# jagannatharjun/AntiZ

Measured on AMD Instinct MI355X. Metric: input MB/s precompressed (1 GB synthetic, 100k streams) at 1/2/4/8 MI355X, higher is better.
Workload: dtype u8

## Files before the change

antiz_amd/__init__.py:

```python
import ctypes as C
import os

HERE = os.path.dirname(os.path.abspath(__file__))
LIB_PATH = os.environ.get("ATZ_LIB") or os.path.join(HERE, "_build", "libatz_accel.so")
CLI_PATH = os.path.join(HERE, "_build", "uncomp")

u64 = C.c_uint64
u8p = C.POINTER(C.c_uint8)


class Opts(C.Structure):
    _fields_ = [("recomp_tresh", u64), ("sizediff_tresh", u64), ("shortcut_len", u64), ("mismatch_tol", u64),
                ("chunksize", u64), ("brute_window", C.c_int32), ("device", C.c_int32)]


class Cand(C.Structure):
    _fields_ = [("offset", u64), ("comp_len", u64), ("infl_len", u64), ("type", C.c_int32), ("flags", C.c_uint32)]


class Result(C.Structure):
    _fields_ = [("clevel", C.c_uint8), ("window", C.c_uint8), ("memlevel", C.c_uint8), ("recomp", C.c_uint8),
                ("n_trials", C.c_uint32), ("ident", u64), ("first_diff", C.c_int64), ("n_diff", u64),
                ("diff_index", u64)]


class Stats(C.Structure):
    _fields_ = [(k, u64) for k in ("file_bytes", "n_streams", "n_recomp", "n_trials", "n_trials_shortcut",
                                   "n_rounds", "atz_bytes", "n_candidates", "n_continuations", "n_hazard")] + \
               [(k, C.c_double) for k in ("scan_ms", "sweep_ms", "write_ms", "total_ms", "k_trial_ms",
                                          "k_inflate_ms", "k_chains_ms", "k_other_ms")] + \
               [(k, u64) for k in ("k_trial_launches", "k_inflate_launches", "k_chains_launches",
                                   "k_trial_alg_bytes", "k_inflate_alg_bytes", "k_chains_alg_bytes",
                                   "trial_parsed_bytes")] + \
               [("k_match_ms", C.c_double)] + \
               [(k, u64) for k in ("k_match_launches", "k_match_positions", "n_trials_rerun", "n_fast_fallbacks",
                                   "trial_cyc_total", "trial_cyc_tree", "trial_cyc_emit", "trial_blocks",
                                   "trial_cyc_heap", "trial_cyc_fallback", "trial_symbols",
                                   "n_trials_speculative", "n_reinflated", "n_inflate_retries", "n_trials_replayed", "n_replay_checked",
                                   "n_trials_duplicate", "n_fast_restarts", "dev_bytes_peak", "dev_bytes_held",
                                   "n_trials_skipped")]

    def as_dict(self):
        return {k: getattr(self, k) for k, _ in self._fields_}


EXPORTS = ["atz_open", "atz_close", "atz_strerror", "atz_free", "atz_default_opts", "atz_scan", "atz_sweep",
           "atz_precompress", "atz_precompress_device", "atz_reconstruct", "atz_deflate", "atz_deflate_batch",
           "atz_inflate_batch", "atz_deflate_bound", "atz_shard_scan", "atz_shard_sweep", "atz_shard_piece",
           "atz_shard_assemble", "atz_reconstruct_device", "atz_deflate_batch_ex", "atz_set_strategies",
           "atz_set_containers", "atz_container_anchors"]

STRATEGIES = {"filtered": 1, "huffman": 2, "rle": 3}


def strategy_mask(names):
    if isinstance(names, str):
        names = [w for w in names.split(",") if w]
    mask = 0
    for w in names:
        if w not in STRATEGIES:
            raise ValueError("unknown strategy %r (known: %s)" % (w, ", ".join(sorted(STRATEGIES))))
        mask |= 1 << STRATEGIES[w]
    return mask


CONTAINERS = {"zip": 0, "gzip": 1}


def container_mask(names):
    if isinstance(names, str):
        names = [w for w in names.split(",") if w]
    mask = 0
    for w in names:
        if w not in CONTAINERS:
            raise ValueError("unknown container %r (known: %s)" % (w, ", ".join(sorted(CONTAINERS))))
        mask |= 1 << CONTAINERS[w]
    return mask


def pack_clevel(strategy, level, raw=False):
    if not (0 <= strategy <= 3 and 0 <= level <= 9) or (strategy >= 2 and level < 1):
        raise ValueError("strategy %d with level %d" % (strategy, level))
    return (int(bool(raw)) << 6) | (strategy << 4) | level


def unpack_clevel(b):
    return b >> 4, b & 15


def unpack_clevel3(b):
    return bool(b & 0x40), (b >> 4) & 3, b & 15

_lib = None


class AtzError(RuntimeError):

    def __init__(self, msg, code=0):
        super().__init__(msg)
        self.code = code


def lib():
    global _lib
    if _lib is None:
        if not os.path.exists(LIB_PATH):
            raise AtzError("libatz_accel.so not built: run `python -m antiz_amd.build` (no CPU fallback)")
        L = C.CDLL(LIB_PATH)
        L.atz_open.argtypes = [C.POINTER(C.c_void_p), C.POINTER(Opts)]
        L.atz_close.argtypes = [C.c_void_p]
        L.atz_strerror.restype = C.c_char_p
        L.atz_strerror.argtypes = [C.c_int]
        L.atz_free.argtypes = [C.c_void_p]
        L.atz_default_opts.argtypes = [C.POINTER(Opts)]
        L.atz_scan.argtypes = [C.c_void_p, C.c_char_p, u64, C.POINTER(C.POINTER(Cand)), C.POINTER(u64)]
        L.atz_sweep.argtypes = [C.c_void_p, C.POINTER(Cand), u64, C.POINTER(Result), C.POINTER(C.POINTER(u64)),
                                C.POINTER(u8p), C.POINTER(u64)]
        L.atz_precompress.argtypes = [C.c_void_p, C.c_char_p, u64, C.POINTER(u8p), C.POINTER(u64), C.POINTER(Stats)]
        L.atz_precompress_device.argtypes = [C.c_void_p, C.c_void_p, C.c_char_p, u64, C.POINTER(C.c_void_p),
                                             C.POINTER(u64), C.POINTER(Stats)]
        L.atz_reconstruct.argtypes = [C.c_void_p, C.c_char_p, u64, C.POINTER(u8p), C.POINTER(u64)]
        L.atz_deflate.argtypes = [C.c_void_p, C.c_char_p, u64, C.c_int, C.c_int, C.c_int, C.c_char_p, u64,
                                  C.POINTER(u64)]
        L.atz_inflate_batch.argtypes = [C.c_void_p, C.c_char_p, u64, C.POINTER(u64), C.POINTER(u64), u64,
                                        C.POINTER(C.c_uint32), C.POINTER(u64), C.POINTER(u64)]
        L.atz_deflate_batch.argtypes = [C.c_void_p, C.c_char_p, u64, C.POINTER(u64), C.POINTER(u64),
                                        C.POINTER(C.c_uint32), u64, C.c_char_p, C.POINTER(u64), C.POINTER(u64),
                                        C.POINTER(u64)]
        L.atz_deflate_batch_ex.argtypes = L.atz_deflate_batch.argtypes
        L.atz_set_strategies.argtypes = [C.c_void_p, C.c_uint32]
        L.atz_set_containers.argtypes = [C.c_void_p, C.c_uint32]
        L.atz_container_anchors.argtypes = [C.c_void_p, C.c_char_p, u64, C.c_uint32, C.POINTER(C.POINTER(u64)),
                                            C.POINTER(u64)]
        L.atz_deflate_bound.restype = u64
        L.atz_deflate_bound.argtypes = [u64, C.c_int, C.c_int]
        L.atz_shard_scan.argtypes = [C.c_void_p, C.c_void_p, C.c_char_p, u64, C.c_int, C.c_int, C.POINTER(u8p),
                                     C.POINTER(u64)]
        L.atz_shard_sweep.argtypes = [C.c_void_p, C.c_void_p, C.c_char_p, u64, C.POINTER(C.c_char_p),
                                      C.POINTER(u64), C.c_int, C.POINTER(u64), C.POINTER(u8p), C.POINTER(u64),
                                      C.POINTER(u64), C.POINTER(Stats)]
        L.atz_shard_piece.argtypes = [C.c_void_p, C.c_void_p]
        L.atz_reconstruct_device.argtypes = [C.c_void_p, C.c_void_p, C.c_char_p, u64, C.POINTER(C.c_void_p),
                                             C.POINTER(u64)]
        L.atz_shard_assemble.argtypes = [C.c_void_p, C.c_void_p, u64, C.c_char_p, u64, u64, u64, C.c_void_p, u64,
                                         C.POINTER(u64)]
        _lib = L
    return _lib


def _check(rc):
    if rc != 0:
        raise AtzError("atz error %d: %s" % (rc, lib().atz_strerror(rc).decode()), rc)


class Context:

    def __init__(self, recomp_tresh=128, sizediff_tresh=128, shortcut_len=512, mismatch_tol=2,
                 chunksize=524288, brute_window=False, device=-1, strategies=None, containers=None):
        L = lib()
        self.o = Opts(recomp_tresh, sizediff_tresh, shortcut_len, mismatch_tol, chunksize, int(brute_window), device)
        if strategies is None:
            strategies = os.environ.get("ATZ_STRATEGIES", "")
        mask = strategy_mask(strategies)
        if containers is None:
            containers = os.environ.get("ATZ_CONTAINERS", "")
        cmask = container_mask(containers)
        self.h = C.c_void_p()
        _check(L.atz_open(C.byref(self.h), C.byref(self.o)))
        if mask:
            _check(L.atz_set_strategies(self.h, mask))
        if cmask:
            _check(L.atz_set_containers(self.h, cmask))

    def close(self):
        if self.h:
            lib().atz_close(self.h)
            self.h = C.c_void_p()

    def __enter__(self):
        return self

    def __exit__(self, *a):
        self.close()

    def precompress(self, data):
        L = lib()
        p = u8p()
        n = u64(0)
        st = Stats()
        _check(L.atz_precompress(self.h, data, len(data), C.byref(p), C.byref(n), C.byref(st)))
        out = C.string_at(p, n.value)
        L.atz_free(p)
        return out, st.as_dict()
# ... 137 lines not shown
```

antiz_amd/csrc/atz_accel.cpp:

```cpp
#include "k_inflate.hip"
#include "k_deflate.hip"

#include <algorithm>
#include <array>
#include <chrono>
#include <cstdio>
#include <cstdlib>
#include <cstring>
#include <deque>
#include <string>
#include <memory>
#include <new>
#include <stdexcept>
#include <atomic>
#include <thread>
#include <condition_variable>
#include <mutex>
#include <functional>
#include <unordered_map>
#include <vector>
#include <dlfcn.h>
#include <signal.h>
#include <sys/time.h>
#include <ucontext.h>
// ... 164 lines not shown
    if (i < MAXS) pcs()[i] = (uint64_t)((ucontext_t*)uc)->uc_mcontext.gregs[REG_RIP] | ((uint64_t)slot << 56);
  }
  static void enroll() {
    if (!on().load() || my_slot() >= 0) return;
    std::lock_guard<std::mutex> lk(mu());
    const int k = nthr().load();
    if (k >= MAXT) return;
    thr()[k] = pthread_self();
    alive()[k] = true;
    my_slot() = k;
    nthr().store(k + 1);
  }
  static void leave() {
    if (my_slot() < 0) return;
    std::lock_guard<std::mutex> lk(mu());
    alive()[my_slot()] = false;
    my_slot() = -1;
  }
  struct Enroll { Enroll() { enroll(); } ~Enroll() { leave(); } };
  const char* path = nullptr;
  std::thread sampler;
  std::atomic<bool> stop{false};
  HostProf() {
    path = std::getenv("ATZ_HOSTPROF");
    if (!path || !*path) { path = nullptr; return; }
    pcs();
    n().store(0);
    struct sigaction sa{};
    sa.sa_sigaction = on_sig;
    sa.sa_flags = SA_SIGINFO | SA_RESTART;
    sigemptyset(&sa.sa_mask);
    sigaction(SIGPROF, &sa, nullptr);
    {
      std::lock_guard<std::mutex> lk(mu());
      nthr().store(0);
    }
    on().store(true);
    enroll();
    sampler = std::thread([this] {
      while (!stop.load()) {
        {
          std::lock_guard<std::mutex> lk(mu());
          const int k = std::min(nthr().load(), MAXT);
          for (int i = 0; i < k; i++)
            if (alive()[i]) pthread_kill(thr()[i], SIGPROF);
        }
        std::this_thread::sleep_for(std::chrono::microseconds(100));
      }
    });
  }
  ~HostProf() {
    if (!path) return;
    stop.store(true);
    sampler.join();
    on().store(false);
    const size_t cnt = std::min(n().load(), MAXS);
    std::unordered_map<uint64_t, uint64_t> hist;
    for (size_t i = 0; i < cnt; i++) hist[pcs()[i]]++;
    FILE* f = std::fopen(path, "a");
    if (f) {
      std::fprintf(f, "# call: %zu samples, %d threads\n", cnt, nthr().load());
      for (const auto& kv : hist) {
        const uint64_t pc = kv.first & ((1ull << 56) - 1);
        Dl_info di{};
        if (dladdr((void*)(uintptr_t)pc, &di) && di.dli_fname)
          std::fprintf(f, "%llu %d %s 0x%llx %s\n", (unsigned long long)kv.second, (int)(kv.first >> 56), di.dli_fname,
                       (unsigned long long)(pc - (uint64_t)(uintptr_t)di.dli_fbase), di.dli_sname ? di.dli_sname : "?");
        else
          std::fprintf(f, "%llu %d ? 0x%llx ?\n", (unsigned long long)kv.second, (int)(kv.first >> 56), (unsigned long long)pc);
      }
      std::fclose(f);
    }
    leave();
    std::lock_guard<std::mutex> lk(mu());
    nthr().store(0);
  }
};

struct DBuf {
  void* p = nullptr;
  size_t n = 0;
  DBuf() = default;
  DBuf(const DBuf&) = delete;
  DBuf& operator=(const DBuf&) = delete;
  ~DBuf() { release(); }
  int reserve(size_t need) {
    if (need <= n) return 0;
    const auto t0 = std::chrono::steady_clock::now();
    release();
    size_t cap = need + need / 4 + 65536;
    const hipError_t e = hipMalloc(&p, cap);
    g_dev.n_alloc++;
    g_dev.alloc_us += (uint64_t)std::chrono::duration_cast<std::chrono::microseconds>(std::chrono::steady_clock::now() - t0).count();
    if (e != hipSuccess) { p = nullptr; return ATZ_E_NOMEM; }
    n = cap;
    g_dev.add(n);
    return 0;
  }
  void release() {
    if (p) { hipFree(p); g_dev.sub(n); g_dev.n_free++; }
    p = nullptr;
    n = 0;
  }
  template <typename T> T* as() const { return reinterpret_cast<T*>(p); }
};

struct PinBuf {
  void* p = nullptr;
  size_t n = 0;
  PinBuf() = default;
  PinBuf(const PinBuf&) = delete;
  PinBuf& operator=(const PinBuf&) = delete;
  ~PinBuf() { if (p) (void)hipHostFree(p); }
  int reserve(size_t need) {
    if (need <= n) return 0;
    const auto t0 = std::chrono::steady_clock::now();
    if (p) { (void)hipHostFree(p); g_dev.n_free++; }
    p = nullptr;
    n = 0;
    const hipError_t e = hipHostMalloc(&p, need, hipHostMallocDefault);
    g_dev.n_alloc++;
    g_dev.alloc_us += (uint64_t)std::chrono::duration_cast<std::chrono::microseconds>(std::chrono::steady_clock::now() - t0).count();
    if (e != hipSuccess) return ATZ_E_NOMEM;
    n = need;
    return 0;
  }
  template <typename T> T* as() const { return reinterpret_cast<T*>(p); }
};

struct Rec {
  uint64_t offset, comp_len, infl_len;
  int type;
  uint32_t flags;
  uint64_t arena_off = ~0ull;
  bool noshort = false;
  uint8_t mhint = 0;
};

struct StreamState {
  const std::vector<uint32_t>* list = nullptr;
  uint32_t idx = 0;
  uint32_t phase = 0;
  uint8_t c = 9, w = 15, m = 9;
  uint64_t ident = 0;
  int64_t first_diff = -1;
  std::vector<uint32_t> rawdiff;
  std::vector<uint8_t> diffval;
  uint32_t trials = 0;
  int32_t rp = -1;
  uint16_t rp_saved = 0, rp_busy = 0;
  uint8_t rp_win[10] = {};
  bool recomp = false;
  std::vector<std::array<uint16_t, 5>> xl;
};


uint32_t pk(int c, int w, int m) { return ((uint32_t)c << 16) | ((uint32_t)w << 8) | (uint32_t)m; }

void prange(std::vector<uint32_t>& l, int cmin, int cmax, int wmin, int wmax, int mmin, int mmax) {
  for (int w = wmax; w >= wmin; w--)
    for (int m = mmax; m >= mmin; m--)
      for (int c = cmax; c >= cmin; c--) l.push_back(pk(c, w, m));
}
void list_a(std::vector<uint32_t>& l, int type) {
  if (type >= 24) return;
  int w = 10 + type / 4;
  switch (type % 4) {
    case 0: l.push_back(pk(0, w, 8)); l.push_back(pk(1, w, 8)); l.push_back(pk(1, w, 9));
            prange(l, 1, 1, w, w, 1, 7); prange(l, 2, 9, w, w, 1, 9); break;
    case 1: prange(l, 2, 5, w, w, 8, 8); prange(l, 2, 5, w, w, 1, 7); prange(l, 2, 5, w, w, 9, 9);
            prange(l, 1, 1, w, w, 1, 9); prange(l, 6, 9, w, w, 1, 9); break;
    case 2: l.push_back(pk(6, w, 8)); l.push_back(pk(6, w, 9)); prange(l, 6, 6, w, w, 1, 7);
            prange(l, 1, 5, w, w, 1, 9); prange(l, 7, 9, w, w, 1, 9); break;
    default: prange(l, 7, 9, w, w, 8, 8); prange(l, 7, 9, w, w, 1, 7); prange(l, 7, 9, w, w, 9, 9);
             prange(l, 1, 6, w, w, 1, 9); break;
  }
}
void list_b(std::vector<uint32_t>& l, int type) {
  if (type >= 24) return;
  int w = 10 + type / 4;
  if (w == 10) prange(l, 1, 9, 11, 15, 1, 9);
  else if (w == 15) prange(l, 1, 9, 10, 14, 1, 9);
  else { prange(l, 1, 9, 10, w - 1, 1, 9); prange(l, 1, 9, w + 1, 15, 1, 9); }
}

const std::vector<uint32_t>& trial_list(int type, bool brute) {
  static const std::array<std::array<std::vector<uint32_t>, 27>, 2> L = [] {
    std::array<std::array<std::vector<uint32_t>, 27>, 2> t;
    for (int ty = 0; ty < 27; ty++) { list_a(t[0][ty], ty); list_b(t[1][ty], ty); }
    return t;
  }();
  return L[brute ? 1 : 0][type];
}

uint64_t bound(uint64_t n, int w, int m) {
  uint64_t complen = n + ((n + 7) >> 3) + ((n + 63) >> 6) + 5;
  if (w != 15 || m + 7 != 15) return complen + 6;
  return n + (n >> 12) + (n >> 14) + (n >> 25) + 13 - 6 + 6;
}

double ms_since(std::chrono::steady_clock::time_point t) {
  return std::chrono::duration<double, std::milli>(std::chrono::steady_clock::now() - t).count();
}

void make_tables(DeflTables& T) {
  static const int xlb[29] = {0,0,0,0,0,0,0,0,1,1,1,1,2,2,2,2,3,3,3,3,4,4,4,4,5,5,5,5,0};
  static const int xdb[30] = {0,0,0,0,1,1,2,2,3,3,4,4,5,5,6,6,7,7,8,8,9,9,10,10,11,11,12,12,13,13};
  std::memset(&T, 0, sizeof(T));
  int len = 0, code;
  for (code = 0; code < 28; code++) {
    T.lbase[code] = (uint16_t)len;
    for (int k = 0; k < (1 << xlb[code]); k++) T.lcode[len++] = (uint8_t)code;
  }
  T.lbase[28] = 0;
  T.lcode[255] = 28;
  int dist = 0;
  for (code = 0; code < 16; code++) {
    T.dbase[code] = (uint16_t)dist;
    for (int k = 0; k < (1 << xdb[code]); k++) T.dcode[dist++] = (uint8_t)code;
  }
  dist >>= 7;
  for (; code < 30; code++) {
    T.dbase[code] = (uint16_t)(dist << 7);
    for (int k = 0; k < (1 << (xdb[code] - 7)); k++) T.dcode[256 + dist++] = (uint8_t)code;
  }
  uint16_t blc[16] = {0};
  for (int n = 0; n < 288; n++) {
    T.st_llen[n] = n < 144 ? 8 : n < 256 ? 9 : n < 280 ? 7 : 8;
    blc[T.st_llen[n]]++;
  }
  uint16_t next[16];
  uint32_t c = 0;
  for (int b = 1; b <= 15; b++) { c = (c + blc[b - 1]) << 1; next[b] = (uint16_t)c; }
  auto rev = [](uint32_t v, int l) { uint32_t r = 0; for (int i = 0; i < l; i++) { r = (r << 1) | (v & 1); v >>= 1; } return r; };
  for (int n = 0; n < 288; n++) T.st_lcode[n] = (uint16_t)rev(next[T.st_llen[n]]++, T.st_llen[n]);
  for (int n = 0; n < 30; n++) { T.st_dlen[n] = 5; T.st_dcode[n] = (uint16_t)rev((uint32_t)n, 5); }
}

int header_type_host(unsigned b0, unsigned b1) {
  static const uint16_t H[24] = {0x2815, 0x2853, 0x2891, 0x28cf, 0x3811, 0x384f, 0x388d, 0x38cb,
                                 0x480d, 0x484b, 0x4889, 0x48c7, 0x5809, 0x5847, 0x5885, 0x58c3,
                                 0x6805, 0x6843, 0x6881, 0x68de, 0x7801, 0x785e, 0x789c, 0x78da};
  unsigned h = (b0 << 8) | b1;
  for (int t = 0; t < 24; t++) if (H[t] == h) return t;
  return -1;
}

const uint8_t* const INFL_BASE = nullptr;
uint32_t* const CHAIN_BASE = nullptr;

}

struct KTimer {
  std::vector<std::pair<hipEvent_t, hipEvent_t>> pending;
  std::vector<int> kind;
  std::vector<hipEvent_t> pool;
  hipEvent_t get() {
    if (!pool.empty()) { hipEvent_t e = pool.back(); pool.pop_back(); return e; }
    hipEvent_t e; (void)hipEventCreate(&e); return e;
  }
};

struct RpEntry {
  uint32_t reads_max = 0;
  uint64_t addr = 0;
  uint64_t tab = 0;
  uint32_t nsym = 0, flags = 0;
  uint8_t state = 0;
  uint8_t window = 0;
  uint8_t memlevel = 0;
};
struct DevArena {
  static constexpr uint64_t CHUNK = 1ull << 30;
  std::mutex mu;
  std::vector<std::unique_ptr<DBuf>> chunks;
  std::vector<std::pair<uint64_t, uint64_t>> span;
  std::unordered_map<uint64_t, std::vector<uint64_t>> freel;
  size_t cur = 0;
  uint64_t used = 0, total = 0, cap = 0;
  uint64_t reused = 0;
  static uint64_t cls(uint64_t bytes) { return (bytes + 4095) & ~4095ull; }
  void reset(uint64_t cap_) {
    std::lock_guard<std::mutex> lk(mu);
    cur = 0; used = 0; total = 0; cap = cap_; reused = 0;
    freel.clear();
  }
  void release(uint64_t a, uint64_t bytes) {
    std::lock_guard<std::mutex> lk(mu);
    freel[cls(bytes)].push_back(a);
  }
  uint64_t alloc(uint64_t bytes) {
    bytes = cls(bytes);
    std::lock_guard<std::mutex> lk(mu);
    auto it = freel.find(bytes);
    if (it != freel.end() && !it->second.empty()) {
      const uint64_t a = it->second.back();
      it->second.pop_back();
      reused += bytes;
      return a;
    }
    if (total + bytes > cap) return 0;
    while (cur < chunks.size() && used + bytes > chunks[cur]->n) { cur++; used = 0; }
    if (cur == chunks.size()) {
      auto b = std::make_unique<DBuf>();
      if (b->reserve(std::max(CHUNK, bytes)) != 0) { (void)hipGetLastError(); return 0; }
      span.push_back({(uint64_t)(uintptr_t)b->p, (uint64_t)(uintptr_t)b->p + b->n});
      chunks.push_back(std::move(b));
      used = 0;
    }
    const uint64_t a = (uint64_t)(uintptr_t)chunks[cur]->p + used;
    used += bytes;
    total += bytes;
    return a;
  }
  bool holds(uint64_t a, uint64_t len) {
    std::lock_guard<std::mutex> lk(mu);
    for (const auto& s : span)
      if (a >= s.first && a + len <= s.second) return true;
    return false;
  }
};
struct ChainBufs {
  DBuf d_cjobs, d_cjobs2, d_cjobs3, d_heads, d_heads2;
};
struct Pipe {
  hipStream_t st = nullptr;
  KTimer kt;
  atz_stats_t stats{};
  DBuf d_trials, d_tres, d_out, d_syms, d_R, d_mjobs, d_diffjobs, d_diffpos, d_diffval, d_diffcnt, d_djobs;
  DBuf d_stopj;
  uint32_t* stopj_cur = nullptr;
  uint32_t mw_cap = 2;
  std::vector<std::unique_ptr<DBuf>> d_chains;
  size_t chains_next = 0;
  ChainBufs cb;
  PinBuf stage;
  size_t stage_used = 0;
  uint64_t r_next = 0;
  hipEvent_t ev_built = nullptr;

  hipStream_t pst = nullptr;
  std::vector<std::pair<uint32_t, int>> tmp_chains;
  uint64_t diag_builds = 0;
  std::vector<std::pair<uint32_t, uint32_t>> diag_rt;
  std::vector<uint64_t> diag_path;
  std::vector<uint32_t> diag_ntr;
  std::vector<uint16_t> diag_need;
  std::vector<uint32_t> slot;
  int id = 0;
  double t_list = 0, t_chains = 0, t_trials = 0, t_apply = 0, t_copy = 0, t_sync = 0;
  uint64_t n_copy = 0, n_sync = 0;
  static constexpr int NPH = 13;
  double ph[NPH] = {}, ph_wait[NPH] = {};
  std::chrono::steady_clock::time_point lap_t;
  double lap_w = 0;
  void lap_start() { lap_t = std::chrono::steady_clock::now(); lap_w = t_copy + t_sync; }
  void lap(int i) {
    const auto n = std::chrono::steady_clock::now();
    ph[i] += std::chrono::duration<double, std::milli>(n - lap_t).count();
    ph_wait[i] += t_copy + t_sync - lap_w;
    lap_t = n;
    lap_w = t_copy + t_sync;
  }
  uint64_t kind[3][10][14] = {};
  ~Pipe() {
    if (ev_built) hipEventDestroy(ev_built);
    if (pst) { hipStreamSynchronize(pst); hipStreamDestroy(pst); }
    if (st) { hipStreamSynchronize(st); hipStreamDestroy(st); }
    for (hipEvent_t e : kt.pool) hipEventDestroy(e);
  }
};

struct TrialSet {
  std::vector<Trial> tr[3];
  std::vector<uint32_t> perm[3];
  std::vector<TrialRes> res[3];
  size_t base = 0;
};

struct atz_ctx {
  KTimer kt;
  atz_opts_t o{};
  int dev = 0;
  hipStream_t st = nullptr;
  DBuf d_rec, d_atzin;
  DBuf d_file, d_pos, d_cnt, d_hbase, d_jobs, d_res, d_virt, d_infl, d_chains, d_heads, d_streams, d_trials,
      d_tres, d_out, d_syms, d_adler, d_meta, d_segs, d_atz, d_diffjobs, d_diffpos, d_diffval, d_diffcnt,
      d_cjobs, d_cjobs2, d_cjobs3, d_heads2, d_tmp, d_R, d_mjobs, d_ins, d_arena, d_arena_used;
  std::vector<Rec> recs;
  std::vector<uint64_t> infl_off;
  std::vector<uint32_t> adler;
  const uint8_t* hfile = nullptr;
  uint64_t flen = 0;
  bool scan_valid = false;
  uint32_t strat_mask = 0;
  uint32_t cont_mask = 0;
  bool exact_idents = false;
  std::vector<uint32_t> scan_trailer;
  bool file_on_device = false;
  const uint8_t* dev_file = nullptr;
  atz_stats_t stats{};
  std::vector<std::array<uint64_t, 10>> chain_off;
  DevArena chain_arena;
  DevArena rp_arena;
  std::vector<std::array<RpEntry, 9>> rp_pool;
  std::mutex rp_mu;
  PinBuf depth_pin;
  struct Sched {
    std::mutex mu;
    std::condition_variable cv;
    std::vector<std::deque<uint32_t>> q;
    std::vector<size_t> unfinished;
    bool closed = false;
    bool abort = false;
    std::atomic<size_t> published{0};
  } sched;
  std::vector<std::unique_ptr<Pipe>> pipes;
  std::vector<std::unique_ptr<DBuf>> slabs;
  size_t pipes_running = 1;
  size_t sweep_nmax = 0;
  std::atomic<bool> sweep_abort{false};
  std::shared_ptr<struct ScanState> scan_keep;
  std::function<void(uint64_t)> on_records;
  std::vector<StreamState> ss_keep;
  std::vector<StreamDev> sd_keep;
  struct Shard {
    std::shared_ptr<struct ScanState> S;
    int rank = -1, world = 0;
    uint32_t ja = 0, jb = 0;
    uint64_t F = 0;
    std::vector<std::pair<uint64_t, uint64_t>> all;
    uint64_t piece_len = 0;
    int stage = 0;
    std::chrono::steady_clock::time_point t0;
  } shard;
};

template <class C>
static void kbeg(C* c, int kind, hipStream_t st = nullptr) {
  hipEvent_t a = c->kt.get(), b = c->kt.get();
  (void)hipEventRecord(a, st ? st : c->st);
  c->kt.pending.push_back({a, b});
  c->kt.kind.push_back(kind);
}
template <class C>
static void kend(C* c, hipStream_t st = nullptr) { (void)hipEventRecord(c->kt.pending.back().second, st ? st : c->st); }
template <class C>
static void kcollect(C* c) {
  for (size_t i = 0; i < c->kt.pending.size(); i++) {
    float ms = 0;
    (void)hipEventElapsedTime(&ms, c->kt.pending[i].first, c->kt.pending[i].second);
    switch (c->kt.kind[i]) {
      case 0: c->stats.k_trial_ms += ms; c->stats.k_trial_launches++; break;
      case 1: c->stats.k_inflate_ms += ms; c->stats.k_inflate_launches++; break;
      case 2: c->stats.k_chains_ms += ms; c->stats.k_chains_launches++; break;
      case 4: c->stats.k_match_ms += ms; c->stats.k_match_launches++; break;
      default: c->stats.k_other_ms += ms; break;
    }
    c->kt.pool.push_back(c->kt.pending[i].first);
    c->kt.pool.push_back(c->kt.pending[i].second);
  }
  c->kt.pending.clear();
  c->kt.kind.clear();
}

template <class C> static void copy_timed(C*, double) {}
template <> void copy_timed<Pipe>(Pipe* p, double ms) { p->t_copy += ms; p->n_copy++; }
static bool stage_on() {
  static const bool v = [] { const char* e = std::getenv("ATZ_STAGE"); return !e || std::atoi(e) != 0; }();
  return v;
}
static constexpr size_t STAGE_BYTES = 32u << 20;
template <class C> static const void* staged(C*, const void* h, size_t) { return h; }
template <> const void* staged<Pipe>(Pipe* p, const void* h, size_t n) {
  if (!stage_on() || !n) return h;
  if (!p->stage.p && p->stage.reserve(STAGE_BYTES)) return h;
  const size_t a = (p->stage_used + 255) & ~(size_t)255;
  if (a + n > p->stage.n) return h;
  std::memcpy(static_cast<uint8_t*>(p->stage.p) + a, h, n);
  p->stage_used = a + n;
  return static_cast<uint8_t*>(p->stage.p) + a;
}
static hipError_t pipe_sync(Pipe* p) {
  const auto t = std::chrono::steady_clock::now();
  const hipError_t e = hipStreamSynchronize(p->st);
  if (e == hipSuccess) p->stage_used = 0;
  p->t_sync += std::chrono::duration<double, std::milli>(std::chrono::steady_clock::now() - t).count();
  p->n_sync++;
  return e;
}
static hipError_t pipe_copy(Pipe* p, void* dst, const void* src, size_t n, hipMemcpyKind k) {
  const auto t = std::chrono::steady_clock::now();
  if (k == hipMemcpyHostToDevice) src = staged(p, src, n);
  const hipError_t e = hipMemcpyAsync(dst, src, n, k, p->st);
  copy_timed(p, std::chrono::duration<double, std::milli>(std::chrono::steady_clock::now() - t).count());
  return e;
}
template <class C>
static int upload(C* c, DBuf& b, const void* h, size_t n, size_t slack = 4096) {
  if (int r = b.reserve(n + slack)) return r;
  const auto t = std::chrono::steady_clock::now();
  if (n) HIPCHK(hipMemcpyAsync(b.p, staged(c, h, n), n, hipMemcpyHostToDevice, c->st));
  copy_timed(c, std::chrono::duration<double, std::milli>(std::chrono::steady_clock::now() - t).count());
  return 0;
}

static bool sync_debug() {
  static const int v = [] { const char* e = std::getenv("ATZ_SYNC_DEBUG"); return (int)(e && *e == '1'); }();
  return v == 1;
}
#define KCHECK(name)                                                                            \
  do {                                                                                          \
    hipError_t e_ = hipGetLastError();                                                          \
    if (e_ == hipSuccess && sync_debug()) e_ = hipStreamSynchronize(c->st);                     \
    if (e_ != hipSuccess) {                                                                     \
      std::fprintf(stderr, "atz: kernel %s failed: %s (%s:%d)\n", name, hipGetErrorString(e_), \
                   __FILE__, __LINE__);                                                         \
      return ATZ_E_HIP;                                                                         \
    }                                                                                           \
  } while (0)

struct Chunk {
  uint64_t co;
  uint64_t len;
  uint8_t b0;
  bool b0_file;
};

static constexpr uint64_t ARENA_SLOT = 65536;

static int timing_level() {
  static const int v = [] { const char* e = std::getenv("ATZ_TIMING"); return (int)(e ? std::atoi(e) : 0); }();
  return v;
}
static bool timing_on() { return timing_level() >= 1; }

static int run_inflate_jobs(atz_ctx* c, const uint8_t* d_in, uint8_t* d_out, const std::vector<InfJob>& jobs,
                            std::vector<InfRes>& res, uint64_t arena_cap = 0, bool full_ring = false,
                            bool arena_reset = true, bool raw = false) {
  res.resize(jobs.size());
  if (jobs.empty()) return 0;
  auto ti0 = std::chrono::steady_clock::now();
  if (int r = upload(c, c->d_jobs, jobs.data(), jobs.size() * sizeof(InfJob))) return r;
  if (int r = c->d_res.reserve(jobs.size() * sizeof(InfRes))) return r;
  if (int r = c->d_arena_used.reserve(64)) return r;
  if (arena_cap && arena_reset) {
    if (int r = c->d_arena.reserve(arena_cap)) return r;
    HIPCHK(hipMemsetAsync(c->d_arena_used.p, 0, 8, c->st));
  }
  uint32_t n = (uint32_t)jobs.size();
  bool small = !full_ring;
  for (const InfJob& jb : jobs) small = small && jb.out_off != NO_OUT;
  kbeg(c, 1);
  auto kern = small ? (raw ? k_inflate<INF_RING_SMALL, true> : k_inflate<INF_RING_SMALL>)
                    : (raw ? k_inflate<INF_RING_FULL, true> : k_inflate<INF_RING_FULL>);
  hipLaunchKernelGGL(kern, dim3(n), dim3(64), 0, c->st, d_in, d_out, c->d_jobs.as<InfJob>(), c->d_res.as<InfRes>(), n,
                     c->d_arena.as<uint8_t>(), c->d_arena_used.as<unsigned long long>(), arena_cap);
// ... 782 lines not shown
  }
  std::vector<ChainJob> nine, rest;
  for (const ChainJob& jb : big) ((jb.memlevel == 9 && jb.n < 65536) ? nine : rest).push_back(jb);
  big.swap(rest);
  if (!nine.empty()) {
    const size_t nbs = 4096;
    if (int r = B.d_heads2.reserve(nbs * 65536 * 4)) return r;
    std::vector<ChainJob>& pk = nine;
    for (size_t k = 0; k < pk.size(); k++) pk[k].slot = (uint32_t)(k % nbs);
    if (int r = upload(c, B.d_cjobs3, pk.data(), pk.size() * sizeof(ChainJob))) return r;
    for (size_t b0 = 0; b0 < pk.size();) {
      const size_t nb = std::min(nbs - b0 % nbs, pk.size() - b0);
      kbeg(c, 2);
      hipLaunchKernelGGL(k_buckets_pk<16>, dim3((uint32_t)nb), dim3(256), 0, c->st, INFL_BASE,
                         B.d_cjobs3.as<ChainJob>() + b0, chains, B.d_heads2.as<uint32_t>(),
                         (uint32_t)nb);
      kend(c);
      KCHECK("k_buckets_pk");
      b0 += nb;
    }
  }
  const size_t batch = 4096;
  if (!big.empty() && (int)B.d_heads.reserve(batch * 65536 * 8)) return ATZ_E_NOMEM;
  for (size_t k = 0; k < big.size(); k++) big[k].slot = (uint32_t)(k % batch);
  if (int r = upload(c, B.d_cjobs, big.data(), big.size() * sizeof(ChainJob))) return r;
  for (size_t b0 = 0; b0 < big.size(); b0 += batch) {
    size_t nb = std::min(batch, big.size() - b0);
    kbeg(c, 2);
    hipLaunchKernelGGL(k_buckets, dim3((uint32_t)nb), dim3(64), 0, c->st, INFL_BASE,
                       B.d_cjobs.as<ChainJob>() + b0, chains, B.d_heads.as<uint64_t>(),
                       (uint32_t)nb);
    kend(c);
    KCHECK("k_buckets");
  }
  for (const ChainJob& jb : jobs) c->stats.k_chains_alg_bytes += 9 * jb.n;
  return 0;
}

static void forget_tmp_chains(atz_ctx* x, Pipe* c) {
  for (auto& q : c->tmp_chains) x->chain_off[q.first][q.second] = ~0ull;
  c->tmp_chains.clear();
  c->chains_next = 0;
}
static int ensure_chains_on(atz_ctx* x, Pipe* c, const std::vector<std::pair<uint32_t, int>>& need, ChainBufs& B) {
  auto bytes = [&](uint32_t s) { return 8 * ((x->recs[s].infl_len + 63) & ~63ull); };
  std::vector<ChainJob> jobs;
  std::vector<size_t> tmp;
  uint64_t tmp_bytes = 0;
  for (auto& q : need) {
    uint32_t s = q.first;
    int m = q.second;
    if (x->chain_off[s][m] != ~0ull) continue;
    ChainJob jb;
    jb.infl_off = x->infl_off[s];
    jb.n = x->recs[s].infl_len;
    jb.memlevel = (uint32_t)m;
    jb.slot = 0;
    jb.dslot = 10 * s + (uint32_t)m;
    jb.pad_ = 0;
    const uint64_t a = x->chain_arena.alloc(bytes(s));
    if (a) {
      jb.chain_off = a >> 2;
    } else {
      jb.chain_off = tmp_bytes >> 2;
      tmp_bytes += (bytes(s) + 255) & ~255ull;
      tmp.push_back(jobs.size());
      c->tmp_chains.push_back({s, m});
    }
    x->chain_off[s][m] = jb.chain_off;
    jobs.push_back(jb);
    c->diag_builds++;
  }
  if (jobs.empty()) return 0;
  if (!tmp.empty()) {
    if (c->chains_next == c->d_chains.size()) c->d_chains.emplace_back(new DBuf());
    DBuf& tb = *c->d_chains[c->chains_next++];
    if (int r = tb.reserve(tmp_bytes + 4096)) return r;
    const uint64_t base = (uint64_t)(uintptr_t)tb.p >> 2;
    for (size_t k : tmp) {
      jobs[k].chain_off += base;
      x->chain_off[(uint32_t)(jobs[k].dslot / 10)][jobs[k].memlevel] = jobs[k].chain_off;
    }
  }
  if (int r = build_bucket_jobs(x, c, B, jobs, CHAIN_BASE, true, x->depth_pin.as<uint32_t>())) return r;
  if (bucket_verify()) {
    uint64_t tot = 0;
    std::vector<ChainJob> alt(jobs);
    for (ChainJob& jb : alt) { jb.chain_off = tot; tot += 2 * ((jb.n + 63) & ~63ull); }
    DBuf tmp;
    if (int r = tmp.reserve(tot * 4 + 4096)) return r;
    if (int r = build_bucket_jobs(x, c, B, alt, tmp.as<uint32_t>(), false, nullptr)) return r;
    std::vector<uint32_t> h1(tot), h2(tot);
    for (size_t k = 0; k < jobs.size(); k++)
      HIPCHK(hipMemcpyAsync(h1.data() + alt[k].chain_off, (const void*)(uintptr_t)(jobs[k].chain_off << 2),
                            8 * ((jobs[k].n + 63) & ~63ull), hipMemcpyDeviceToHost, c->st));
    HIPCHK(hipMemcpyAsync(h2.data(), tmp.p, tot * 4, hipMemcpyDeviceToHost, c->st));
    HIPCHK(hipStreamSynchronize(c->st));
    for (size_t k = 0; k < jobs.size(); k++) {
      const uint64_t npad = (alt[k].n + 63) & ~63ull, nh = alt[k].n >= 3 ? alt[k].n - 2 : 0;
      const uint32_t* a = h1.data() + alt[k].chain_off;
      const uint32_t* b2 = h2.data() + alt[k].chain_off;
      uint64_t start = 0, deepest = 0;
      for (uint64_t i = 0; i < nh; i++) {
        if (a[i] != b2[i] || a[npad + i] != b2[npad + i]) {
          std::fprintf(stderr, "atz: bucket mismatch: job %zu n %llu m %u at %llu\n", k, (unsigned long long)alt[k].n,
                       alt[k].memlevel, (unsigned long long)i);
          return ATZ_E_INTERNAL;
        }
        if (b2[npad + i] & BUCKET_FIRST) start = i;
        deepest = std::max(deepest, i - start);
      }
      const uint32_t dsort = x->depth_pin.p ? x->depth_pin.as<uint32_t>()[jobs[k].dslot] : 0u;
      if (x->depth_pin.p && nh && dsort != ~0u && dsort != deepest) {
        std::fprintf(stderr, "atz: deepest bucket mismatch: job %zu n %llu m %u: %u vs %llu\n", k,
                     (unsigned long long)alt[k].n, alt[k].memlevel, dsort, (unsigned long long)deepest);
        return ATZ_E_INTERNAL;
      }
    }
  }
  return 0;
}

static bool big_sweep(const atz_ctx* x) { return x->recs.size() > 16000 || x->pipes_running >= 6; }
static bool mhint_on(const atz_ctx* x) {
  static const int v = [] { const char* e = std::getenv("ATZ_MHINT"); return e ? std::atoi(e) : -1; }();
  return v < 0 ? big_sweep(x) : v != 0;
}
static uint64_t match_prefix(uint64_t n, int memlevel, bool big) {
  static const uint64_t mul = [] { const char* e = std::getenv("ATZ_PREFIX_MUL"); return e ? (uint64_t)std::max(1, std::atoi(e)) : 2ull; }();
  static const uint64_t lo = [] { const char* e = std::getenv("ATZ_PREFIX_MIN"); return e ? (uint64_t)std::max(64, std::atoi(e)) : 0ull; }();
  const uint64_t floor = lo ? lo : big ? 3072 : 1024;
  return std::min(n, std::max<uint64_t>(floor, mul << (memlevel + 6)));
}

static uint32_t lazy_host(uint32_t level) {
  return level == 7 ? 32u : level == 8 ? 128u : 258u;
}
static uint32_t nice_host(uint32_t level) {
  return level == 7 ? 128u : 258u;
}
static uint64_t c_cfg_host(uint32_t level) {
  static const uint16_t chain[10] = {0, 4, 8, 32, 16, 32, 128, 256, 1024, 4096};
  return chain[level < 10 ? level : 9];
}
static uint64_t match_win() {
  static const uint64_t v = [] { const char* e = std::getenv("ATZ_MATCH_WIN"); return e ? (uint64_t)std::atoll(e) : 16320ull; }();
  return v;
}
static uint64_t match_span(const MatchJob& m) {
  const uint64_t md = (1ull << m.window) - 262;
  const uint64_t lo = m.p0 > md ? (m.p0 - md) & ~3ull : 0ull;
  return std::min<uint64_t>(m.p1 + 258 + 24, m.n) - lo;
}
static int launch_match(atz_ctx* x, Pipe* c, const std::vector<MatchJob>& mj_in) {
  if (mj_in.empty()) return 0;
  static const uint64_t cls[] = {4096, 8192, 12288, 16384, 24576, 32768, 40960, 49152};
  constexpr int NC = 8;
  std::vector<MatchJob> cut;
  const bool win = match_win() > 0;
  if (win)
    for (const MatchJob& m : mj_in) {
      if (match_span(m) <= cls[NC - 1]) { cut.push_back(m); continue; }
      for (uint64_t a = m.p0; a < m.p1; a += std::min<uint64_t>(match_win(), 16320)) {
        MatchJob h = m;
        h.p0 = a;
        h.p1 = std::min<uint64_t>(m.p1, a + std::min<uint64_t>(match_win(), 16320));
        cut.push_back(h);
      }
    }
  const std::vector<MatchJob>& mj0 = win ? cut : mj_in;
  auto class_of = [&](const MatchJob& m) -> int {
    const uint64_t b = match_span(m);
    for (int k = 0; k < NC; k++) if (b <= cls[k] && (win || k < 6)) return k;
    return NC;
  };
  auto group_of = [](int k) -> int { return k; };
  std::vector<MatchJob> mj;
  mj.reserve(mj0.size());
  size_t cnt[NC + 1] = {};
  int gmax[NC + 1];
  for (int k = 0; k <= NC; k++) gmax[k] = -1;
  for (const MatchJob& m : mj0) {
    const int k = class_of(m), g = group_of(k);
    cnt[g]++;
    gmax[g] = std::max(gmax[g], k);
  }
  size_t beg[NC + 2] = {};
  for (int k = 0; k <= NC; k++) beg[k + 1] = beg[k] + cnt[k];
  mj.resize(mj0.size());
  {
    size_t at[NC + 1];
    for (int k = 0; k <= NC; k++) at[k] = beg[k];
    for (const MatchJob& m : mj0) mj[at[group_of(class_of(m))]++] = m;
    auto work = [](const MatchJob& m) -> uint64_t {
      const uint64_t chain = std::min<uint64_t>(c_cfg_host(m.level), (m.p1 >> (m.memlevel + 7)) + 1);
      return (m.p1 - m.p0) * chain;
    };
    for (int k = 0; k <= NC; k++)
      std::stable_sort(mj.begin() + beg[k], mj.begin() + beg[k + 1],
                       [&](const MatchJob& a, const MatchJob& b) { return work(a) > work(b); });
  }
  if (int r = upload(c, c->d_mjobs, mj.data(), mj.size() * sizeof(MatchJob))) return r;
  for (int k = 0; k <= NC; k++) {
    if (!cnt[k]) continue;
    kbeg(c, 4);
    if (k < NC)
      hipLaunchKernelGGL(k_match_lds, dim3((uint32_t)cnt[k]), dim3(MATCH_THREADS), (uint32_t)(3 * cls[gmax[k]] + 64), c->st,
                         INFL_BASE, CHAIN_BASE, c->d_R.as<uint2>(),
                         c->d_mjobs.as<MatchJob>() + beg[k]);
    else
      hipLaunchKernelGGL(k_match, dim3((uint32_t)cnt[k]), dim3(256), 0, c->st, INFL_BASE,
                         CHAIN_BASE, c->d_R.as<uint2>(), c->d_mjobs.as<MatchJob>() + beg[k]);
    kend(c);
    KCHECK("k_match");
  }
  for (const MatchJob& m : mj) c->stats.k_match_positions += m.p1 - m.p0;
  return 0;
}

static uint32_t mw_cap_for(size_t n_streams) {
  static const int v = [] { const char* e = std::getenv("ATZ_MW"); return (int)(e ? std::max(0, std::min(9, std::atoi(e))) : -1); }();
  return v >= 0 ? (uint32_t)v : n_streams <= 16000 ? 4u : 2u;
}
static bool mw_trial(const Pipe* c, int kind, uint32_t memlevel) { return kind != 0 && memlevel <= c->mw_cap; }
static uint32_t trial_variant(const Pipe* c, int k, const Trial& t) {
  return (mw_trial(c, k, t.memlevel) ? 1u : 0u) | ((t.host & TH_STRAT) << 1);
}
static uint64_t sym_words(const Pipe* c, int kind, uint32_t memlevel, uint64_t n) {
  return (mw_trial(c, kind, memlevel) ? n + 64 : 0) + (1ull << (memlevel + 6)) + 64;
}
struct TrialBatch {
  std::vector<Trial> tr[3];
  uint64_t out_tot = 0, sym_tot = 0;
  std::pair<int, uint32_t> add(const Pipe* c, uint32_t s, uint64_t len, int cl, int w, int m, uint32_t strat,
                               uint8_t mode, uint64_t best_ident) {
    if (strat == 1 && cl < 4) strat = 0;
    const int kind = cl == 0 || strat >= 2 ? 0 : cl <= 3 ? 1 : 2;
    Trial t{};
    t.stream = s; t.clevel = (uint8_t)cl; t.window = (uint8_t)w; t.memlevel = (uint8_t)m;
    t.mode = mode; t.host = strat;
    t.best_ident = best_ident;
    t.out_off = out_tot; t.out_cap = bound(len, w, m) + 64;
    out_tot += (t.out_cap + 255) & ~255ull;
    t.sym_off = sym_tot; sym_tot += sym_words(c, kind, (uint32_t)m, len);
    tr[kind].push_back(t);
    return {kind, (uint32_t)tr[kind].size() - 1};
  }
  int reserve(Pipe* c) const {
    if (int r = c->d_out.reserve(out_tot + 4096)) return r;
    return c->d_syms.reserve(sym_tot * 4 + 4096);
  }
};

static bool stopflag_on() {
  static const bool v = [] { const char* e = std::getenv("ATZ_STOPFLAG"); return !e || std::atoi(e) != 0; }();
  return v;
}
static void trials_order(atz_ctx* x, const Pipe* c, std::vector<Trial>* in, TrialSet& S) {
  for (int k = 0; k < 3; k++) {
    const size_t n = in[k].size();
    S.perm[k].resize(n);
    std::vector<uint64_t> key(n);
    const uint32_t mwm = c->mw_cap;
    const bool packed = n < (1u << 20);
    bool strat = false;
    for (size_t q = 0; q < n; q++) {
      const Trial& t = in[k][q];
      strat |= (t.host & TH_STRAT) != 0;
      const uint64_t w = x->recs[t.stream].infl_len * (uint64_t)(k == 1 ? 3 : 1) * (uint64_t)(10 - t.memlevel) *
                         (uint64_t)((t.mode & TM_REPLAY) ? 1 : 4);
      const uint64_t mw = k != 0 && t.memlevel <= mwm;
      const uint64_t jr = stopflag_on() ? 15 - std::min<uint32_t>(t.spec_j, 15) : 0;
      key[q] = packed ? (mw << 63) | (jr << 59) | (std::min<uint64_t>(w, (1ull << 39) - 1) << 20) | ((1u << 20) - 1 - q) : w;
      S.perm[k][q] = (uint32_t)q;
    }
    if (packed) {
      std::sort(key.begin(), key.end(), std::greater<uint64_t>());
      for (size_t q = 0; q < n; q++) S.perm[k][q] = (uint32_t)((1u << 20) - 1 - (key[q] & ((1u << 20) - 1)));
    } else {
      std::stable_sort(S.perm[k].begin(), S.perm[k].end(), [&](uint32_t a, uint32_t b) {
        const bool ma = mw_trial(c, k, in[k][a].memlevel), mb = mw_trial(c, k, in[k][b].memlevel);
        return ma != mb ? ma : key[a] > key[b];
      });
    }
    if (strat)
      std::stable_sort(S.perm[k].begin(), S.perm[k].end(), [&](uint32_t a, uint32_t b) {
        return trial_variant(c, k, in[k][a]) < trial_variant(c, k, in[k][b]);
      });
    S.tr[k].resize(n);
    for (size_t q = 0; q < n; q++) S.tr[k][q] = in[k][S.perm[k][q]];
    S.res[k].clear();
  }
  S.base = 0;
}
static int trials_launch(atz_ctx* x, Pipe* c, const uint8_t* d_cmp, const SweepOpts& so, int k, const Trial* h,
                         size_t cnt, size_t base) {
  struct Kern { int kind; uint32_t strat; bool mw; void (*fn)(SweepArgs); const char* name; };
  static const Kern kerns[] = {
      {0, 0, false, k_trial_stored, "k_trial_stored"},
      {0, 2, false, k_trial_huff, "k_trial_huff"},
      {0, 3, false, k_trial_rle, "k_trial_rle"},
      {1, 0, true, k_trial_fast_mw<BITMAP_BITS>, "k_trial_fast"},
      {1, 0, false, k_trial_fast<BITMAP_BITS>, "k_trial_fast"},
      {2, 0, true, k_trial_slow_mw, "k_trial_slow"},
      {2, 0, false, k_trial_slow, "k_trial_slow"},
      {2, 1, true, k_trial_slow_filt_mw, "k_trial_slow_filt"},
      {2, 1, false, k_trial_slow_filt, "k_trial_slow_filt"},
  };
  for (size_t i = 0; i < cnt; i++)
    if (h[i].host & (TH_WAITS | TH_DUP)) return ATZ_E_INTERNAL;
  for (size_t i = 0; i < cnt;) {
    const bool mw = mw_trial(c, k, h[i].memlevel);
    size_t j = i + 1;
    while (j < cnt && mw_trial(c, k, h[j].memlevel) == mw) j++;
    HIPCHK(pipe_copy(c, c->d_trials.as<Trial>() + base + i, h + i, (j - i) * sizeof(Trial), hipMemcpyHostToDevice));
    i = j;
  }
  auto launch1 = [&](const Trial* hh, size_t n1, size_t b1, uint32_t variant) -> int {
    (void)hh;
    const bool mw = variant & 1u;
    const Kern* kn = nullptr;
    for (const Kern& e : kerns)
      if (e.kind == k && e.strat == variant >> 1 && e.mw == mw) kn = &e;
    if (!kn) return ATZ_E_INTERNAL;
    SweepArgs A;
    A.file = d_cmp; A.infl = INFL_BASE; A.chains = CHAIN_BASE;
    A.R = c->d_R.as<uint2>();
    A.streams = x->d_streams.as<StreamDev>(); A.trials = c->d_trials.as<Trial>() + b1;
    A.res = c->d_tres.as<TrialRes>() + b1; A.out = c->d_out.as<uint8_t>(); A.syms = c->d_syms.as<uint32_t>();
    A.adler = x->d_adler.as<uint32_t>(); A.o = so; A.ntrials = (uint32_t)n1;
    A.stopj = c->stopj_cur;
    dim3 g((uint32_t)n1), b(mw ? MW_THREADS : 64);
    kbeg(c, 0);
    hipLaunchKernelGGL(kn->fn, g, b, 0, c->st, A);
    kend(c);
    KCHECK(kn->name);
    return 0;
  };
  size_t i = 0;
  while (i < cnt) {
    const uint32_t v = trial_variant(c, k, h[i]);
    size_t j = i + 1;
    while (j < cnt && trial_variant(c, k, h[j]) == v) j++;
    if (int r = launch1(h + i, j - i, base + i, v)) return r;
    i = j;
  }
  return 0;
}
static bool early_match_on() {
  static const bool v = [] { const char* e = std::getenv("ATZ_EARLY"); return !e || std::atoi(e) != 0; }();
  return v;
}
static MatchJob first_match_job(atz_ctx* x, Pipe* c, int k, Trial& t) {
  const uint64_t n = x->recs[t.stream].infl_len;
  t.r_off = c->r_next;
  c->r_next += ((n + 63) & ~63ull) + 256;
  t.x_lim = (t.mode & TM_FULL) || (mhint_on(x) && t.memlevel == x->recs[t.stream].mhint) ? n : match_prefix(n, t.memlevel, big_sweep(x));
  MatchJob m{};
  m.infl_off = x->infl_off[t.stream]; m.n = n; m.chain_off = t.chain_off; m.r_off = t.r_off;
  m.p0 = 0; m.p1 = t.x_lim; m.level = t.clevel; m.window = t.window; m.fast = k == 1; m.memlevel = t.memlevel;
  return m;
}
static int trials_first_launch(atz_ctx* x, Pipe* c, const uint8_t* d_cmp, TrialSet& S, const SweepOpts& so,
                               size_t bases[3]) {
  std::vector<Trial>* tr = S.tr;
  std::vector<TrialRes>* res = S.res;
  std::vector<MatchJob> mj;
  for (int k = 0; k < 3; k++)
    for (const Trial& t : tr[k])
      if (x->recs[t.stream].infl_len >= (1ull << 31)) {
        std::fprintf(stderr, "atz: stream of %llu inflated bytes exceeds the 2 GiB trial limit\n",
                     (unsigned long long)x->recs[t.stream].infl_len);
        return ATZ_E_ARG;
      }
  for (int k = 1; k < 3; k++)
    for (Trial& t : tr[k]) {
      const uint64_t n = x->recs[t.stream].infl_len;
      if (tm_unchecked_replay(t.mode)) { t.r_off = 0; t.x_lim = n; continue; }
      if (t.x_lim) continue;
      if (MatchJob m = first_match_job(x, c, k, t); m.p1 > m.p0) mj.push_back(m);
    }
  if (int r = c->d_R.reserve(c->r_next * sizeof(uint2) + 4096)) return r;
  c->lap(6);
  if (int r = launch_match(x, c, mj)) return r;
  c->lap(7);
  const size_t tot_trials = tr[0].size() + tr[1].size() + tr[2].size();
  if (int r = c->d_trials.reserve(2 * tot_trials * sizeof(Trial) + 64)) return r;
  if (int r = c->d_tres.reserve(2 * tot_trials * sizeof(TrialRes) + 64)) return r;
  size_t base = 0;
  for (int k = 0; k < 3; k++) {
    bases[k] = base;
    res[k].resize(tr[k].size());
    if (tr[k].empty()) continue;
    if (int r = trials_launch(x, c, d_cmp, so, k, tr[k].data(), tr[k].size(), base)) return r;
    base += tr[k].size();
  }
  S.base = base;
  c->lap(8);
  return 0;
}
static int trials_first_finish(Pipe* c, TrialSet& S, const size_t bases[3]);
static int trials_first(atz_ctx* x, Pipe* c, const uint8_t* d_cmp, TrialSet& S, const SweepOpts& so) {
  size_t bases[3];
  if (int r = trials_first_launch(x, c, d_cmp, S, so, bases)) return r;
  return trials_first_finish(c, S, bases);
}
static int trials_first_finish(Pipe* c, TrialSet& S, const size_t bases[3]) {
  std::vector<Trial>* tr = S.tr;
  std::vector<TrialRes>* res = S.res;
  for (int k = 0; k < 3; k++)
    if (!tr[k].empty())
      HIPCHK(pipe_copy(c, res[k].data(), c->d_tres.as<TrialRes>() + bases[k], tr[k].size() * sizeof(TrialRes), hipMemcpyDeviceToHost));
  HIPCHK(pipe_sync(c));
  kcollect(c);
  c->lap(9);
  return 0;
}
static int trials_rerun(atz_ctx* x, Pipe* c, const uint8_t* d_cmp, TrialSet& S, const SweepOpts& so,
                        const std::function<bool(const Trial&)>& want) {
  std::vector<Trial>* tr = S.tr;
  std::vector<TrialRes>* res = S.res;
  std::vector<Trial> again[3];
  std::vector<size_t> where[3];
  std::vector<MatchJob> mj;
  for (int k = 1; k < 3; k++)
    for (size_t q = 0; q < tr[k].size(); q++) {
      if (res[k][q].state != TR_NEED_R || (want && !want(tr[k][q]))) continue;
      Trial t = tr[k][q];
      const uint64_t n = x->recs[t.stream].infl_len;
      MatchJob m{};
      m.infl_off = x->infl_off[t.stream]; m.n = n; m.chain_off = t.chain_off; m.r_off = t.r_off;
      m.p0 = t.x_lim; m.p1 = n; m.level = t.clevel; m.window = t.window; m.fast = k == 1; m.memlevel = t.memlevel;
      if (m.p1 > m.p0) mj.push_back(m);
      t.x_lim = n;
      again[k].push_back(t);
      where[k].push_back(q);
      c->stats.n_trials_rerun++;
    }
  if (again[1].empty() && again[2].empty()) return 0;
  if (int r = launch_match(x, c, mj)) return r;
  std::vector<TrialRes> rr[3];
  size_t base = S.base, bases[3] = {0, 0, 0};
  if (base + again[1].size() + again[2].size() > 2 * (tr[0].size() + tr[1].size() + tr[2].size())) return ATZ_E_INTERNAL;
  for (int k = 1; k < 3; k++) {
    bases[k] = base;
    if (again[k].empty()) continue;
    if (int r = trials_launch(x, c, d_cmp, so, k, again[k].data(), again[k].size(), base)) return r;
    rr[k].resize(again[k].size());
    base += again[k].size();
  }
  for (int k = 1; k < 3; k++)
    if (!again[k].empty())
      HIPCHK(pipe_copy(c, rr[k].data(), c->d_tres.as<TrialRes>() + bases[k], again[k].size() * sizeof(TrialRes), hipMemcpyDeviceToHost));
  HIPCHK(pipe_sync(c));
  kcollect(c);
  for (int k = 1; k < 3; k++)
    for (size_t q = 0; q < again[k].size(); q++) {
      if (rr[k][q].state == TR_NEED_R) return ATZ_E_INTERNAL;
      res[k][where[k][q]] = rr[k][q];
      tr[k][where[k][q]].x_lim = again[k][q].x_lim;
    }
  S.base = base;
  return 0;
}
static void trials_results(const TrialSet& S, std::vector<TrialRes>* res) {
  for (int k = 0; k < 3; k++) {
    res[k].resize(S.tr[k].size());
    for (size_t q = 0; q < S.tr[k].size(); q++) res[k][S.perm[k][q]] = S.res[k][q];
  }
}
static int run_trials(atz_ctx* x, Pipe* c, const uint8_t* d_cmp, std::vector<Trial>* tr, const SweepOpts& so,
                      std::vector<TrialRes>* res) {
  TrialSet S;
  trials_order(x, c, tr, S);
  c->r_next = 0;
  if (int r = trials_first(x, c, d_cmp, S, so)) return r;
  if (int r = trials_rerun(x, c, d_cmp, S, so, nullptr)) return r;
  trials_results(S, res);
  return 0;
}

static int replay_mode() {
  static const int v = [] { const char* e = std::getenv("ATZ_REPLAY"); return (int)(e ? std::atoi(e) : 1); }();
  return v;
}
static bool replay_on() { return replay_mode() != 0; }
static constexpr uint64_t RP_ARENA_CAP = 24ull << 30;

static bool dedup_on() {
  static const int v = [] { const char* e = std::getenv("ATZ_DEDUP"); return (int)(e ? std::atoi(e) : 1); }();
  return v != 0;
}
static void replay_from(Trial& t, const RpEntry& e, bool bf) {
  if (bf) {
    t.mode |= TM_REPLAY;
    const uint32_t lm = std::min<uint32_t>(e.memlevel, t.memlevel);
    if (dedup_on() && (uint64_t)e.nsym + 2 <= (1ull << (lm + 6))) t.host |= TH_DUP;
  } else if (e.tab) {
    t.mode |= TM_REPLAY | TM_CHECKED;
    t.rp_tab = e.tab;
  } else {
    return;
  }
  t.rp_syms = e.addr; t.rp_nsym = e.nsym; t.rp_flags = e.flags;
}
static bool budget_free(atz_ctx* x, int kind, const Trial& t) {
  const uint32_t Bq = (uint32_t)(c_cfg_host(t.clevel) >> (kind == 1 ? 0 : 2));
  return x->depth_pin.as<uint32_t>()[10 * (size_t)t.stream + t.memlevel] <= Bq;
}
static bool replay_free(atz_ctx* x, int kind, const Trial& t) {
  return x->recs[t.stream].infl_len <= (1ull << t.window) - 262 && budget_free(x, kind, t);
}

static bool budget_free(atz_ctx* x, int kind, const Trial& t);
static void level_dups(atz_ctx* x, std::vector<StreamState>& ss, std::vector<Trial>& slow) {
  for (Trial& t : slow) {
    if (t.clevel < 7 || t.clevel > 9 || (t.mode & TM_FULL)) continue;
    const StreamState& st = ss[t.stream];
    for (const auto& r : st.xl) {
      if (r[0] != t.window || r[1] != t.memlevel || r[2] <= t.clevel) continue;
      if (r[3] < lazy_host(t.clevel) && r[4] < nice_host(t.clevel) && budget_free(x, 2, t)) t.host |= TH_DUP;
      break;
    }
  }
}
template <class Mine>
static void level_record(atz_ctx* x, std::vector<StreamState>& ss, const std::vector<Trial>& slow,
                         const std::vector<TrialRes>& res, const Mine& mine) {
  for (size_t q = 0; q < slow.size(); q++) {
    const Trial& t = slow[q];
    const TrialRes& r = res[q];
    if (!mine(t.stream)) continue;
    if (t.clevel < 7 || t.clevel > 9 || (t.host & TH_DUP) || r.state == TR_NEED_R || r.state == TR_OVERFLOW ||
        r.state == TR_SKIPPED)
      continue;
    if (!budget_free(x, 2, t)) continue;
    StreamState& st = ss[t.stream];
    bool have = false;
    for (const auto& e : st.xl) have |= e[0] == t.window && e[1] == t.memlevel;
    if (have) continue;
    uint32_t rm = r.reads_max;
    if (r.saved_flags & 4) {
      if (st.rp < 0) continue;
      rm = x->rp_pool[st.rp][t.clevel - 1].reads_max;
    }
    st.xl.push_back({(uint16_t)t.window, (uint16_t)t.memlevel, (uint16_t)t.clevel, (uint16_t)(rm >> 16),
                     (uint16_t)(rm & 0xffffu)});
  }
}

static void plan_replay(atz_ctx* x, Pipe* c, std::vector<StreamState>& ss, int kind, std::vector<Trial>& trs,
                        std::vector<std::array<uint32_t, 4>>& savers) {
  const bool checked = replay_mode() != 3 && kind == 2;
  for (size_t q = 0; q < trs.size(); q++) {
    Trial& t = trs[q];
    if (t.clevel < 1 || t.clevel > 9 || (t.mode & TM_FULL) || (t.host & TH_DUP)) continue;
    const uint64_t n = x->recs[t.stream].infl_len;
    const uint64_t wsz = 1ull << t.window;
    if (n > wsz + (wsz - 262)) continue;
    const bool bf = replay_free(x, kind, t);
    if (!bf && !checked) continue;
    StreamState& st = ss[t.stream];
    const uint32_t L = t.clevel;
    const bool saved = (st.rp_saved >> L) & 1u, busy = (st.rp_busy >> L) & 1u;
    const bool same_w = st.rp_win[L] == t.window;
    if (saved && same_w) {
      if (replay_mode() == 2) continue;
      replay_from(t, x->rp_pool[st.rp][L - 1], bf);
    } else if (busy && same_w && replay_mode() != 2 && (bf || x->rp_pool[st.rp][L - 1].tab)) {
      t.host |= TH_WAITS;
    } else if (!saved && !busy && bf) {
      if (st.rp < 0) {
        std::lock_guard<std::mutex> lk(x->rp_mu);
        if (x->rp_pool.size() == x->rp_pool.capacity()) continue;
        st.rp = (int32_t)x->rp_pool.size();
        x->rp_pool.emplace_back();
      }
      RpEntry& e = x->rp_pool[st.rp][L - 1];
      const uint64_t sb = (4 * (n + 64) + 255) & ~255ull, tb = kind == 2 ? ((8 * n + 255) & ~255ull) : 0;
      if (!e.addr) {
        e.addr = x->rp_arena.alloc(sb + tb);
        if (!e.addr) continue;
        e.tab = tb ? e.addr + sb : 0;
      }
      e.state = 1;
// ... 13 lines not shown
  static const bool on = [] { const char* e = std::getenv("ATZ_ELIG"); return !e || std::atoi(e) != 0; }();
  if (!on || x->exact_idents || x->o.mismatch_tol > x->o.recomp_tresh || C <= x->o.recomp_tresh) return 0;
  return C - x->o.recomp_tresh - 1;
}

static constexpr uint64_t ROUND_BUDGET_BYTES = 24ull << 30;

static bool sched_take(atz_ctx* x, int g, std::vector<uint32_t>& batch) {
  auto& Q = x->sched;
  std::unique_lock<std::mutex> lk(Q.mu);
  batch.clear();
  auto stop = [&] { return Q.abort || x->sweep_abort.load(std::memory_order_relaxed); };
  std::deque<uint32_t>& q = Q.q[g];
  Q.cv.wait(lk, [&] { return stop() || !q.empty() || (Q.closed && Q.unfinished[g] == 0); });
  if (stop() || q.empty()) return false;
  batch.assign(q.begin(), q.end());
  q.clear();
  return true;
}
static void sched_give(atz_ctx* x, int g, const std::vector<StreamState>& ss, const std::vector<uint32_t>& active,
                       const std::vector<uint32_t>& waiting) {
  auto& Q = x->sched;
  std::lock_guard<std::mutex> lk(Q.mu);
  std::vector<uint32_t> front(waiting);
  size_t done = 0;
  for (uint32_t s : active) { if (ss[s].phase == 2) done++; else front.push_back(s); }
  Q.unfinished[g] -= done;
  Q.q[g].insert(Q.q[g].begin(), front.begin(), front.end());
  Q.cv.notify_all();
}
static void sched_abort(atz_ctx* x) {
  std::lock_guard<std::mutex> lk(x->sched.mu);
  x->sched.abort = true;
  x->sched.cv.notify_all();
}

static size_t round_target(const atz_ctx* x);
static void account_trial(atz_ctx* x, Pipe* c, int k, const Trial& t, const TrialRes& r) {
  const uint64_t C = x->recs[t.stream].comp_len;
  c->stats.trial_parsed_bytes += r.parsed;
  c->stats.n_fast_fallbacks += r.fallbacks & 0xffffffffull;
  c->stats.n_fast_restarts += r.fallbacks >> 32;
  c->stats.n_trials_skipped += r.state == TR_SKIPPED;
  c->stats.trial_cyc_total += r.cyc_total; c->stats.trial_cyc_tree += r.cyc_tree;
  c->stats.trial_cyc_emit += r.cyc_emit; c->stats.trial_blocks += r.blocks;
  c->stats.trial_cyc_heap += r.cyc_heap; c->stats.trial_cyc_fallback += r.cyc_fallback;
  c->stats.trial_symbols += r.symbols;
  uint64_t* gk = c->kind[k][t.clevel];
  gk[0]++; gk[1] += r.cyc_total; gk[2] += r.cyc_tree; gk[3] += r.cyc_emit; gk[4] += r.cyc_heap;
  gk[5] += r.cyc_fallback; gk[6] += r.parsed; gk[7] += r.symbols; gk[8] += r.cyc_scan; gk[9] += r.cyc_send;
  for (int i = 0; i < 4; i++) gk[10 + i] += r.cyc_sec[i];
  if (!(t.host & TH_DUP))
    c->stats.k_trial_alg_bytes += r.state == TR_NEED_R || r.state == TR_SKIPPED ? r.parsed
                                  : x->recs[t.stream].infl_len + (r.out_len < C ? r.out_len : C);
  if (timing_level() >= 3 && !(t.host & TH_DUP)) {
    c->diag_rt.push_back({r.rt0, r.rt1});
    if (c->diag_path.size() <= t.stream) { c->diag_path.resize(x->recs.size(), 0); c->diag_ntr.resize(x->recs.size(), 0); }
    c->diag_path[t.stream] += (uint32_t)(r.rt1 - r.rt0);
    c->diag_ntr[t.stream]++;
  }
}
static int private_chains(atz_ctx* c, Pipe* p, const std::vector<std::pair<uint32_t, int>>& need) {
  for (auto& a : c->chain_off) a.fill(~0ull);
  c->chain_arena.reset(cap_bytes(CHAIN_CACHE_CAP));
  p->tmp_chains.clear();
  p->chains_next = 0;
  if (int r = ensure_chains(c, p, need)) return r;
  HIPCHK(hipStreamSynchronize(p->st));
  return 0;
}

struct RuleTally { uint64_t ntr = 0, nsc = 0, nhz = 0; };
struct RuleStep { bool improved = false, stop = false, diff = false; };
static int rule_step(const atz_opts_t& o, uint64_t C, const TrialRes& r, uint64_t& best, RuleTally& n, RuleStep& out) {
  n.ntr++;
  if (r.state == TR_SHORTCUT) n.nsc++;
  if (r.flags & 1) n.nhz++;
  if (r.state == TR_OVERFLOW) return ATZ_E_REF_ABORT;
  out = RuleStep{};
  if (r.state == TR_FULL && r.ident > best) {
    best = r.ident;
    out.improved = true;
    out.stop = r.ident == C || r.ident + o.mismatch_tol >= C;
    out.diff = r.ident != C && C - r.ident <= o.recomp_tresh;
  }
  return 0;
}

static int run_diffs(Pipe* c, const uint8_t* d_file, std::vector<DiffJob>& dj, std::vector<std::vector<uint32_t>>& pos,
                     std::vector<std::vector<uint8_t>>& val) {
  pos.assign(dj.size(), {});
  val.assign(dj.size(), {});
  if (dj.empty()) return 0;
  uint64_t dpos = 0;
  for (DiffJob& d : dj) { d.dst = dpos; dpos += d.cap; }
  if (int r = upload(c, c->d_diffjobs, dj.data(), dj.size() * sizeof(DiffJob))) return r;
  if (int r = c->d_diffpos.reserve(dpos * 4 + 64)) return r;
  if (int r = c->d_diffval.reserve(dpos + 64)) return r;
  if (int r = c->d_diffcnt.reserve(dj.size() * 8 + 64)) return r;
  kbeg(c, 3);
  hipLaunchKernelGGL(k_diffs, dim3((uint32_t)dj.size()), dim3(64), 0, c->st, c->d_out.as<uint8_t>(), d_file,
                     c->d_diffjobs.as<DiffJob>(), c->d_diffpos.as<uint32_t>(), c->d_diffval.as<uint8_t>(),
                     c->d_diffcnt.as<uint64_t>(), (uint32_t)dj.size());
  kend(c);
  KCHECK("k_diffs");
  std::vector<uint32_t> hp(dpos);
  std::vector<uint8_t> hv(dpos);
  std::vector<uint64_t> cnt(dj.size());
  HIPCHK(pipe_copy(c, hp.data(), c->d_diffpos.p, dpos * 4, hipMemcpyDeviceToHost));
  HIPCHK(pipe_copy(c, hv.data(), c->d_diffval.p, dpos, hipMemcpyDeviceToHost));
  HIPCHK(pipe_copy(c, cnt.data(), c->d_diffcnt.p, dj.size() * 8, hipMemcpyDeviceToHost));
  HIPCHK(pipe_sync(c));
  kcollect(c);
  for (size_t q = 0; q < dj.size(); q++) {
    if (cnt[q] != dj[q].cap) return ATZ_E_INTERNAL;
    pos[q].assign(hp.begin() + dj[q].dst, hp.begin() + dj[q].dst + dj[q].cap);
    val[q].assign(hv.begin() + dj[q].dst, hv.begin() + dj[q].dst + dj[q].cap);
  }
  return 0;
}

struct Round : TrialBatch {
  atz_ctx* x; Pipe* c; const uint8_t* d_file; std::vector<StreamState>& ss; const SweepOpts& so;
  std::vector<uint32_t>& active;
  std::vector<uint32_t>& waiting;
  uint32_t K = 1;
  std::vector<TrialRes> trres[3];
  std::vector<std::pair<int, uint32_t>> mine;
  std::vector<uint32_t> mbeg;
  std::vector<std::pair<uint32_t, int>> need;
  std::vector<uint32_t> need_b;
  std::vector<std::array<uint32_t, 4>> savers;
  uint64_t r_bound = 0;
  size_t nbuild = 0;
  std::vector<uint8_t> held;
  TrialSet SA, SB;
  std::vector<uint32_t> ia[3], ib[3];
  bool waiting_trials = false;
  struct PendDiff { bool live = false; DiffJob d{}; };
  std::vector<PendDiff> pend;
  std::vector<uint32_t> jpos;
  RuleTally tally;
  uint64_t nspec = 0;

  Round(atz_ctx* x_, Pipe* c_, const uint8_t* f, std::vector<StreamState>& ss_, const SweepOpts& so_,
        std::vector<uint32_t>& a_, std::vector<uint32_t>& w_)
      : x(x_), c(c_), d_file(f), ss(ss_), so(so_), active(a_), waiting(w_) {}

  bool is_held(uint32_t s) const { return held[c->slot[s]] != 0; }

  void build_lists() {
    K = (uint32_t)std::max<size_t>(1, std::min<size_t>(32, round_target(x) / active.size()));
    c->mw_cap = mw_cap_for(std::min(x->sweep_nmax, active.size() * x->pipes_running));
    mbeg.assign(active.size() + 1, 0);
    mine.reserve(active.size() * K);
    uint64_t round_bytes = 0;
    const uint64_t round_budget = cap_bytes(ROUND_BUDGET_BYTES) / x->pipes_running;
    for (size_t a = 0; a < active.size(); a++) {
      mbeg[a] = (uint32_t)mine.size();
      const uint32_t s = active[a];
      StreamState& st = ss[s];
      if (a > 0 && round_bytes > round_budget) {
        waiting.insert(waiting.begin(), active.begin() + a, active.end());
        active.resize(a);
        break;
      }
      for (uint32_t j = 0; j < K && st.idx + j < st.list->size(); j++) {
        const uint32_t p = (*st.list)[st.idx + j];
        const int cl = (int)(p >> 16), w = (int)((p >> 8) & 0xff), m = (int)(p & 0xff);
        const uint64_t len = x->recs[s].infl_len;
        const auto at = add(c, s, len, cl, w, m, 0, 0, st.ident);
        const int kind = at.first;
        Trial& t = tr[kind][at.second];
        t.spec_j = j;
        round_bytes += 8 * (len + 320) + t.out_cap + 4 * sym_words(c, kind, (uint32_t)m, len);
        if (kind) {
          r_bound += ((len + 63) & ~63ull) + 256;
          need.push_back({s, m});
          need_b.push_back((uint32_t)(c_cfg_host((uint32_t)cl) >> (kind == 1 ? 0 : 2)));
        }
        mine.push_back(at);
      }
    }
    mbeg.resize(active.size() + 1);
    mbeg[active.size()] = (uint32_t)mine.size();
    held.assign(active.size(), 0);
    if (c->slot.size() < x->recs.size()) c->slot.resize(x->recs.size());
    for (size_t a = 0; a < active.size(); a++) c->slot[active[a]] = (uint32_t)a;
    pend.assign(active.size(), PendDiff{});
    jpos.assign(mbeg.begin(), mbeg.end() - 1);
  }

  int plan() {
    c->r_next = 0;
    if (int r = c->d_R.reserve(r_bound * sizeof(uint2) + 4096)) return r;
    c->stopj_cur = nullptr;
    if (K > 1 && stopflag_on()) {
      if (int r = c->d_stopj.reserve(x->recs.size() * sizeof(uint32_t) + 64)) return r;
      HIPCHK(hipMemsetAsync(c->d_stopj.p, 0xff, x->recs.size() * sizeof(uint32_t), c->st));
      c->stopj_cur = c->d_stopj.as<uint32_t>();
    }
    if (replay_on() && x->depth_pin.p) {
      std::vector<std::pair<uint32_t, int>> dfirst, direct;
      std::vector<uint32_t> dfirst_b;
      std::vector<std::pair<int, uint32_t>> early;
      for (int k = 1; k < 3; k++) {
        uint32_t cur = ~0u;
        uint16_t seen[16] = {};
        for (uint32_t q = 0; q < tr[k].size(); q++) {
          const Trial& t = tr[k][q];
          if (t.stream != cur) { cur = t.stream; std::memset(seen, 0, sizeof seen); }
          const bool again = (seen[t.window & 15] >> t.clevel) & 1u;
          seen[t.window & 15] |= (uint16_t)(1u << t.clevel);
          const StreamState& st = ss[t.stream];
          bool maybe = false;
          if (st.rp >= 0) maybe = ((st.rp_saved >> t.clevel) & 1u) && st.rp_win[t.clevel] == t.window;
          if (!maybe && k == 2 && t.clevel >= 7)
            for (const auto& r : st.xl) maybe |= r[0] == t.window && r[1] == t.memlevel && r[2] > t.clevel;
          static const bool all_first = [] { const char* e = std::getenv("ATZ_DFIRST"); return e && std::atoi(e) == 0; }();
          if (maybe || all_first) {
            dfirst.push_back({t.stream, (int)t.memlevel});
            dfirst_b.push_back((uint32_t)(c_cfg_host(t.clevel) >> (k == 1 ? 0 : 2)));
          } else {
            direct.push_back({t.stream, (int)t.memlevel});
            if (!again) early.push_back({k, q});
          }
        }
      }
      for (auto& q : direct) nbuild += x->chain_off[q.first][q.second] == ~0ull;
      if (int r = ensure_depths(x, c, dfirst, dfirst_b, c->d_djobs)) return r;
      if (int r = ensure_chains(x, c, direct)) return r;
      c->lap(1);
      if (early_match_on() && !early.empty()) {
        if (!c->ev_built) HIPCHK(hipEventCreateWithFlags(&c->ev_built, hipEventDisableTiming));
        HIPCHK(hipEventRecord(c->ev_built, c->st));
        std::vector<MatchJob> mj;
        mj.reserve(early.size());
        for (const auto& e : early) {
          Trial& t = tr[e.first][e.second];
          t.chain_off = x->chain_off[t.stream][t.memlevel];
          if (MatchJob m = first_match_job(x, c, e.first, t); m.p1 > m.p0) mj.push_back(m);
        }
        if (int r = launch_match(x, c, mj)) return r;
        c->lap(6);
        const auto t_ev = std::chrono::steady_clock::now();
        HIPCHK(hipEventSynchronize(c->ev_built));
        c->t_sync += ms_since(t_ev);
        c->n_sync++;
      } else {
        HIPCHK(pipe_sync(c));
      }
      c->lap(2);
      if (dedup_on()) level_dups(x, ss, tr[2]);
      for (int k = 1; k < 3; k++) plan_replay(x, c, ss, k, tr[k], savers);
      c->lap(3);
      need.clear();
      for (int k = 1; k < 3; k++)
        for (const Trial& t : tr[k])
          if (!tm_unchecked_replay(t.mode) && !(t.host & TH_DUP)) need.push_back({t.stream, (int)t.memlevel});
    }
    for (int k = 0; k < 3; k++)
      for (Trial& t : tr[k])
        if (!(t.mode & TM_SAVE)) t.best_ident = std::max(t.best_ident, elig_floor(x, x->recs[t.stream].comp_len));
    for (auto& q : need) nbuild += x->chain_off[q.first][q.second] == ~0ull;
    if (int r = ensure_chains(x, c, need)) return r;
    for (int k = 1; k < 3; k++)
      for (Trial& t : tr[k]) {
        const uint64_t off = x->chain_off[t.stream][t.memlevel];
        t.chain_off = off == ~0ull ? 0 : off;
      }
    for (int k = 1; k < 3; k++)
      for (const Trial& t : tr[k])
        if ((t.mode & TM_RP_SYMS) && !replay_slot_ok(t)) return ATZ_E_INTERNAL;
    if (int r = reserve(c)) return r;
    c->lap(4);
    return 0;
  }
  bool replay_slot_ok(const Trial& t) const {
    const uint64_t n = x->recs[t.stream].infl_len;
    const bool syms_ok = !(t.mode & TM_RP_SYMS) || x->rp_arena.holds(t.rp_syms, 4 * (n + 64));
    const bool tab_ok = !(t.mode & TM_RP_TAB) || x->rp_arena.holds(t.rp_tab, 8 * n);
    if (syms_ok && tab_ok && !((t.mode & TM_REPLAY) && t.rp_nsym > n)) return true;
    std::fprintf(stderr, "atz: symbol replay slot out of its arena (stream %u)\n", t.stream);
    return false;
  }

  void finish_savers(bool held_ones) {
    for (const auto& sv : savers) {
      if (is_held(tr[sv[0]][sv[1]].stream) != held_ones) continue;
      const TrialRes& r = trres[sv[0]][sv[1]];
      RpEntry& e = x->rp_pool[sv[2]][sv[3]];
      StreamState& st = ss[tr[sv[0]][sv[1]].stream];
      const uint16_t bit = (uint16_t)(1u << (sv[3] + 1));
      st.rp_busy &= (uint16_t)~bit;
      if (r.state != TR_NEED_R && r.state != TR_SKIPPED && (r.saved_flags & 1u)) {
        e.state = 2; e.nsym = r.saved_syms; e.flags = r.saved_flags; e.reads_max = r.reads_max;
        st.rp_saved |= bit;
      } else {
        e.state = 0;
      }
    }
  }
  void collect(const TrialSet& S, const std::vector<uint32_t>* idx) {
    std::vector<TrialRes> rr[3];
    trials_results(S, rr);
    for (int k = 0; k < 3; k++)
      for (size_t j = 0; j < idx[k].size(); j++) trres[k][idx[k][j]] = rr[k][j];
  }

  int launch() {
    TrialRes dup{};
    dup.state = TR_CANT_BEAT;
    for (int k = 1; k < 3; k++)
      for (const Trial& t : tr[k]) waiting_trials |= (t.host & TH_WAITS) != 0;
    {
      std::vector<Trial> ta[3];
      for (int k = 0; k < 3; k++) {
        trres[k].assign(tr[k].size(), dup);
        for (uint32_t q = 0; q < tr[k].size(); q++) {
          if (tr[k][q].host & (TH_WAITS | TH_DUP)) continue;
          ta[k].push_back(tr[k][q]);
          ia[k].push_back(q);
        }
      }
      trials_order(x, c, ta, SA);
    }
    c->lap(5);
    {
      size_t bases[3];
      if (int r = trials_first_launch(x, c, d_file, SA, so, bases)) return r;
      if (int r = trials_first_finish(c, SA, bases)) return r;
    }
    if (!waiting_trials) {
      collect(SA, ia);
      return 0;
    }
    if (int r = trials_rerun(x, c, d_file, SA, so, nullptr)) return r;
    collect(SA, ia);
    finish_savers(false);
    std::vector<Trial> t3[3];
    for (int k = 1; k < 3; k++)
      for (uint32_t q = 0; q < tr[k].size(); q++) {
        Trial& t = tr[k][q];
        if (!(t.host & TH_WAITS)) continue;
        t.host &= ~TH_WAITS;
        const RpEntry& e = x->rp_pool[ss[t.stream].rp][t.clevel - 1];
        if (e.state == 2 && e.window == t.window) replay_from(t, e, replay_free(x, k, t));
        if (t.host & TH_DUP) continue;
        if ((t.mode & TM_REPLAY) && !replay_slot_ok(t)) return ATZ_E_INTERNAL;
        t3[k].push_back(t);
        ib[k].push_back(q);
      }
    trials_order(x, c, t3, SB);
    if (int r = trials_first(x, c, d_file, SB, so)) return r;
    collect(SB, ib);
    return 0;
  }

  int walk(size_t a, bool defer) {
    const uint32_t s = active[a];
    StreamState& st = ss[s];
    const uint64_t C = x->recs[s].comp_len;
    const uint32_t phase0 = st.phase;
    held[a] = 0;
    for (uint32_t j = jpos[a]; j < mbeg[a + 1]; j++) {
      if (st.phase != phase0) { nspec += mbeg[a + 1] - j; break; }
      const Trial& t = tr[mine[j].first][mine[j].second];
      const TrialRes& r = trres[mine[j].first][mine[j].second];
      if (r.state == TR_NEED_R) {
        if (!defer) return ATZ_E_INTERNAL;
        jpos[a] = j;
        held[a] = 1;
        return 0;
      }
      if (r.state == TR_SKIPPED) return ATZ_E_INTERNAL;
      st.trials++;
      RuleStep step;
      if (int e = rule_step(x->o, C, r, st.ident, tally, step)) return e;
      if (step.improved) {
        st.c = t.clevel; st.w = t.window; st.m = t.memlevel;
        st.first_diff = -1;
        st.rawdiff.clear(); st.diffval.clear();
        pend[a].live = step.diff;
        if (step.diff) pend[a].d = DiffJob{t.out_off, r.out_len, x->recs[s].offset, C, 0, C - r.ident};
      }
      st.idx++;
      if (step.stop) st.idx = (uint32_t)st.list->size();
      if (st.idx >= st.list->size()) {
        if (st.phase == 0 && (C - st.ident) >= x->o.mismatch_tol && x->o.brute_window) {
          st.list = &trial_list(x->recs[s].type, true);
          st.idx = 0;
          st.phase = 1;
        } else {
          st.phase = 2;
        }
      }
    }
    jpos[a] = mbeg[a + 1];
    return 0;
  }

  void settle(bool held_ones) {
    finish_savers(held_ones);
    if (dedup_on() && x->depth_pin.p)
      level_record(x, ss, tr[2], trres[2], [&](uint32_t s) { return is_held(s) == held_ones; });
  }

  int apply() {
    for (size_t a = 0; a < active.size(); a++)
      if (int r = walk(a, true)) return r;
    settle(false);
    bool any_held = false;
    for (uint8_t h : held) any_held |= h != 0;
    if (!any_held) return 0;
    auto want = [&](const Trial& t) { return is_held(t.stream); };
    if (int r = trials_rerun(x, c, d_file, SA, so, want)) return r;
    collect(SA, ia);
    if (waiting_trials) {
      if (int r = trials_rerun(x, c, d_file, SB, so, want)) return r;
      collect(SB, ib);
    }
    for (size_t a = 0; a < active.size(); a++)
      if (held[a]) {
        held[a] = 0;
        if (int r = walk(a, false)) return r;
        held[a] = 1;
      }
    settle(true);
    return 0;
  }

  void release_done() {
    for (uint32_t s : active) {
      if (ss[s].phase != 2) continue;
      const uint64_t bytes = 8 * ((x->recs[s].infl_len + 63) & ~63ull);
      for (int m = 1; m <= 9; m++) {
        uint64_t& off = x->chain_off[s][m];
        if (off == ~0ull) continue;
        if (x->chain_arena.holds(off << 2, bytes)) x->chain_arena.release(off << 2, bytes);
        off = ~0ull;
      }
    }
  }

  int flush_diffs() {
    std::vector<DiffJob> dj;
    std::vector<size_t> dja;
    for (size_t a = 0; a < active.size(); a++) {
      if (!pend[a].live) continue;
      pend[a].live = false;
      dj.push_back(pend[a].d);
      dja.push_back(a);
    }
    std::vector<std::vector<uint32_t>> pos;
    std::vector<std::vector<uint8_t>> val;
    if (int r = run_diffs(c, d_file, dj, pos, val)) return r;
    for (size_t q = 0; q < dj.size(); q++) {
      StreamState& st = ss[active[dja[q]]];
      st.rawdiff.swap(pos[q]); st.diffval.swap(val[q]);
      st.first_diff = st.rawdiff.empty() ? -1 : (int64_t)st.rawdiff[0];
    }
    return 0;
  }

  void account(uint64_t round) {
    for (int k = 1; k < 3; k++)
      for (size_t q = 0; q < tr[k].size(); q++) {
        c->stats.n_trials_replayed += (trres[k][q].saved_flags >> 2) & 1u;
        c->stats.n_replay_checked += (tr[k][q].mode & TM_CHECKED) != 0;
        c->stats.n_trials_duplicate += (tr[k][q].host & TH_DUP) != 0;
        if (timing_on() && !tm_unchecked_replay(tr[k][q].mode) && !(tr[k][q].host & TH_DUP)) {
          if (c->diag_need.size() <= tr[k][q].stream) c->diag_need.resize(tr[k][q].stream + 1, 0);
          c->diag_need[tr[k][q].stream] |= (uint16_t)(1u << tr[k][q].memlevel);
        }
      }
    for (int k = 0; k < 3; k++)
      for (size_t q = 0; q < tr[k].size(); q++) account_trial(x, c, k, tr[k][q], trres[k][q]);
    if (!timing_on()) return;
    if (timing_level() >= 3) {
      std::vector<uint32_t> st0, en;
      for (int k = 0; k < 3; k++)
        for (size_t q = 0; q < tr[k].size(); q++)
          if (!(tr[k][q].host & TH_DUP) && trres[k][q].rt1) { st0.push_back(trres[k][q].rt0); en.push_back(trres[k][q].rt1); }
      if (!en.empty()) {
        const uint32_t b = *std::min_element(st0.begin(), st0.end());
        std::sort(en.begin(), en.end());
        auto q = [&](double f) { return (en[std::min(en.size() - 1, (size_t)(f * (double)en.size()))] - b) / 100.0; };
        std::fprintf(stderr, "atz: pipe %d round %llu ends (us after the first start): n %zu p50 %.0f p90 %.0f p95 %.0f p98 %.0f p99 %.0f max %.0f\n",
                     c->id, (unsigned long long)round, en.size(), q(0.5), q(0.9), q(0.95), q(0.98), q(0.99), q(1.0));
      }
    }
    std::vector<std::pair<uint64_t, std::pair<int, size_t>>> top;
    for (int k = 0; k < 3; k++)
      for (size_t q = 0; q < tr[k].size(); q++) top.push_back({trres[k][q].cyc_total, {k, q}});
    std::sort(top.begin(), top.end(), [](auto& p1, auto& p2) { return p1.first > p2.first; });
    for (size_t i = 0; i < top.size() && i < 3; i++) {
      const Trial& t = tr[top[i].second.first][top[i].second.second];
      const TrialRes& r = trres[top[i].second.first][top[i].second.second];
      std::fprintf(stderr, "atz: round %llu slow trial: stream %u I=%llu c%u w%u m%u state %u cyc %.1fM syms %llu blocks %llu "
                   "fallbacks %llu tree %.1fM emit %.1fM (heap %.1fM scan %.1fM send %.1fM fb %.1fM)\n", (unsigned long long)round, t.stream,
                   (unsigned long long)x->recs[t.stream].infl_len, t.clevel, t.window, t.memlevel, r.state,
                   r.cyc_total / 1e6, (unsigned long long)r.symbols, (unsigned long long)r.blocks,
                   (unsigned long long)(r.fallbacks & 0xffffffffull), r.cyc_tree / 1e6, r.cyc_emit / 1e6, r.cyc_heap / 1e6,
                   r.cyc_scan / 1e6, r.cyc_send / 1e6, r.cyc_fallback / 1e6);
    }
  }
};

static int sweep_pipe(atz_ctx* x, Pipe* c, const uint8_t* d_file, std::vector<StreamState>& ss) {
  const auto t0 = std::chrono::steady_clock::now();
  std::vector<uint32_t> active;
  const SweepOpts so{x->o.recomp_tresh, x->o.sizediff_tresh, x->o.shortcut_len, x->o.mismatch_tol};
  uint64_t rounds = 0;
  while (sched_take(x, c->id, active)) {
    rounds++;
    std::vector<uint32_t> waiting;
    struct Give {
      atz_ctx* x; Pipe* c; const std::vector<StreamState>& ss; const std::vector<uint32_t>& a, &w;
      ~Give() {
        c->stopj_cur = nullptr;
        forget_tmp_chains(x, c);
        sched_give(x, c->id, ss, a, w);
      }
    } give{x, c, ss, active, waiting};
    Round R(x, c, d_file, ss, so, active, waiting);
    const auto tl0 = std::chrono::steady_clock::now();
    c->lap_start();
    R.build_lists();
    c->lap(0);
    const auto ta = std::chrono::steady_clock::now();
    if (int r = R.plan()) return r;
    const auto tb = std::chrono::steady_clock::now();
    if (int r = R.launch()) return r;
    const auto tc = std::chrono::steady_clock::now();
    if (int r = R.apply()) return r;
    c->lap(10);
    if (int r = R.flush_diffs()) return r;
    R.release_done();
    c->lap(11);
    const auto td = std::chrono::steady_clock::now();
    c->t_chains += std::chrono::duration<double, std::milli>(tb - ta).count();
    c->t_trials += std::chrono::duration<double, std::milli>(tc - tb).count();
    if (timing_level() >= 2)
      std::fprintf(stderr, "atz: pipe %d round %llu at %.1f ms: active %zu K %u trials %zu/%zu/%zu list %.1f chains %.1f (%zu builds) trials %.1f ms, reruns+apply %.1f ms\n",
                   c->id, (unsigned long long)rounds, std::chrono::duration<double, std::milli>(ta - t0).count(), active.size(), R.K,
                   R.tr[0].size(), R.tr[1].size(), R.tr[2].size(), std::chrono::duration<double, std::milli>(ta - tl0).count(),
                   std::chrono::duration<double, std::milli>(tb - ta).count(), R.nbuild,
                   std::chrono::duration<double, std::milli>(tc - tb).count(),
                   std::chrono::duration<double, std::milli>(td - tc).count());
    R.account(rounds);
    c->lap(12);
    c->t_apply += ms_since(tc);
    c->stats.n_trials += R.tally.ntr; c->stats.n_trials_shortcut += R.tally.nsc; c->stats.n_hazard += R.tally.nhz;
    c->stats.n_trials_speculative += R.nspec;
  }
  c->stats.n_rounds = rounds;
  c->stats.sweep_ms = ms_since(t0);
  return 0;
}

static int ensure_pipes(atz_ctx* c, size_t np) {
  while (c->pipes.size() < np) {
    std::unique_ptr<Pipe> p(new Pipe());
    p->id = (int)c->pipes.size();
    if (hipStreamCreateWithFlags(&p->st, hipStreamNonBlocking) != hipSuccess) return ATZ_E_HIP;
    if (hipStreamCreateWithFlags(&p->pst, hipStreamNonBlocking) != hipSuccess) return ATZ_E_HIP;
    c->pipes.push_back(std::move(p));
  }
  return 0;
}
static size_t sweep_pipes(size_t n) {
  static const std::pair<int, int> cfg = [] {
    const char* e = std::getenv("ATZ_PIPES");
    const char* q = std::getenv("GPU_MAX_HW_QUEUES");
    return std::make_pair(e ? std::max(1, std::min(8, std::atoi(e))) : -1, q ? std::atoi(q) : 4);
  }();
  if (cfg.first > 0) return (size_t)cfg.first;
  return n <= 16000 && cfg.second >= 8 ? 6 : 3;
}
static size_t round_target(const atz_ctx* x) {
  static const int env = [] { const char* e = std::getenv("ATZ_TARGET"); return e ? std::max(256, std::atoi(e)) : 0; }();
  if (env) return (size_t)env;
  return x->sched.published.load() <= 32000 ? 8192 : 4096;
}
struct SweepRun {
  const uint8_t* d_file = nullptr;
  std::vector<StreamState>* ss = nullptr;
  size_t np = 0, published = 0;
  std::vector<StreamDev> sd;
  std::vector<std::thread> th;
  std::vector<int> rc;
  std::chrono::steady_clock::time_point t0;
  bool running = false;
};

static void sweep_close(atz_ctx* c, SweepRun& R, bool abort = false) {
  {
    std::lock_guard<std::mutex> lk(c->sched.mu);
    c->sched.closed = true;
    if (abort) c->sched.abort = true;
    c->sched.cv.notify_all();
  }
  for (auto& t : R.th) t.join();
  R.th.clear();
  R.running = false;
}

static int sweep_begin(atz_ctx* c, const uint8_t* d_file, std::vector<StreamState>& ss, size_t n_max, SweepRun& R) {
  R.t0 = std::chrono::steady_clock::now();
  R.d_file = d_file;
  R.ss = &ss;
  R.published = 0;
  ss.assign(n_max, StreamState());
  c->chain_off.assign(n_max, {});
  for (auto& a : c->chain_off) a.fill(~0ull);
  c->chain_arena.reset(cap_bytes(CHAIN_CACHE_CAP));
  c->rp_arena.reset(cap_bytes(RP_ARENA_CAP));
  c->rp_pool.clear();
  c->rp_pool.reserve(n_max);
  if (int r = c->depth_pin.reserve(n_max * 40 + 64)) return r;
  std::memset(c->depth_pin.p, 0xff, n_max * 40);
  if (c->infl_off.size() < n_max) c->infl_off.resize(n_max);
  if (c->adler.size() < n_max) c->adler.resize(n_max);
  R.sd.assign(n_max, StreamDev{});
  if (int r = c->d_adler.reserve(n_max * 4 + 4096)) return r;
  if (int r = c->d_streams.reserve(n_max * sizeof(StreamDev) + 4096)) return r;
  R.np = std::max<size_t>(1, std::min(sweep_pipes(n_max), (n_max + 255) / 256));
  c->pipes_running = R.np;
  c->sweep_nmax = n_max;
  if (int r = ensure_pipes(c, R.np)) return r;
  {
    auto& Q = c->sched;
    std::lock_guard<std::mutex> lk(Q.mu);
    Q.q.assign(R.np, std::deque<uint32_t>());
    Q.unfinished.assign(R.np, 0);
    Q.closed = false;
    Q.abort = false;
    Q.published = 0;
  }
  for (size_t g = 0; g < R.np; g++) {
    Pipe* p = c->pipes[g].get();
    p->tmp_chains.clear();
    p->stats = atz_stats_t{};
    p->t_list = p->t_chains = p->t_trials = p->t_apply = p->t_copy = p->t_sync = 0;
    p->n_copy = p->n_sync = 0;
    std::memset(p->ph, 0, sizeof(p->ph));
    std::memset(p->ph_wait, 0, sizeof(p->ph_wait));
    std::memset(p->kind, 0, sizeof(p->kind));
  }
  R.rc.assign(R.np, 0);
  R.running = true;
  for (size_t g = 0; g < R.np; g++)
    R.th.emplace_back([c, &R, &ss, g]() {
      if (hipSetDevice(c->dev) != hipSuccess) { R.rc[g] = ATZ_E_HIP; sched_abort(c); return; }
      HostProf::Enroll prof_enroll;
      try {
        R.rc[g] = sweep_pipe(c, c->pipes[g].get(), R.d_file, ss);
      } catch (const std::bad_alloc&) {
        R.rc[g] = ATZ_E_NOMEM;
      } catch (...) {
        R.rc[g] = ATZ_E_INTERNAL;
      }
      if (R.rc[g]) sched_abort(c);
    });
  return 0;
}

static int sweep_publish(atz_ctx* c, SweepRun& R, size_t r0, size_t r1) {
  if (r1 <= r0) return 0;
  if (r1 > R.sd.size()) return ATZ_E_INTERNAL;
  for (size_t s = r0; s < r1; s++) {
    StreamDev& d = R.sd[s];
    d.orig_off = c->recs[s].offset; d.infl_off = c->infl_off[s];
    d.comp_len = c->recs[s].comp_len; d.infl_len = c->recs[s].infl_len;
    (*R.ss)[s].list = &trial_list(c->recs[s].type, false);
  }
  HIPCHK(hipMemcpyAsync(c->d_adler.as<uint32_t>() + r0, c->adler.data() + r0, (r1 - r0) * 4, hipMemcpyHostToDevice, c->st));
  HIPCHK(hipMemcpyAsync(c->d_streams.as<StreamDev>() + r0, R.sd.data() + r0, (r1 - r0) * sizeof(StreamDev),
                        hipMemcpyHostToDevice, c->st));
  HIPCHK(hipStreamSynchronize(c->st));
  {
    auto& Q = c->sched;
    std::lock_guard<std::mutex> lk(Q.mu);
    for (size_t s = r0; s < r1; s++) {
      if (c->recs[s].type >= 24) { (*R.ss)[s].phase = 2; continue; }
      Q.q[s % R.np].push_back((uint32_t)s); Q.unfinished[s % R.np]++;
    }
    Q.published = r1;
    Q.cv.notify_all();
  }
  R.published = r1;
  return 0;
}

static int sweep_finish(atz_ctx* c, SweepRun& R) {
  sweep_close(c, R);
  const size_t np = R.np, n = R.published;
  std::vector<StreamState>& ss = *R.ss;
  for (size_t g = 0; g < np; g++) if (R.rc[g]) return R.rc[g];
  ss.resize(n);
  uint64_t kind[3][10][14] = {};
  double tch = 0, ttr = 0, tap = 0;
  for (size_t g = 0; g < np; g++) {
    const Pipe* p = c->pipes[g].get();
    const atz_stats_t& q = p->stats;
    atz_stats_t& t = c->stats;
    t.n_trials += q.n_trials; t.n_trials_shortcut += q.n_trials_shortcut; t.n_hazard += q.n_hazard;
    t.n_rounds = std::max(t.n_rounds, q.n_rounds); t.n_trials_speculative += q.n_trials_speculative;
    t.k_trial_ms += q.k_trial_ms; t.k_chains_ms += q.k_chains_ms; t.k_other_ms += q.k_other_ms; t.k_match_ms += q.k_match_ms;
    t.k_trial_launches += q.k_trial_launches; t.k_chains_launches += q.k_chains_launches;
    t.k_match_launches += q.k_match_launches;
    t.k_trial_alg_bytes += q.k_trial_alg_bytes; t.k_chains_alg_bytes += q.k_chains_alg_bytes;
    t.trial_parsed_bytes += q.trial_parsed_bytes; t.k_match_positions += q.k_match_positions;
    t.n_trials_rerun += q.n_trials_rerun; t.n_fast_fallbacks += q.n_fast_fallbacks; t.n_fast_restarts += q.n_fast_restarts;
    t.trial_cyc_total += q.trial_cyc_total; t.trial_cyc_tree += q.trial_cyc_tree; t.trial_cyc_emit += q.trial_cyc_emit;
    t.trial_blocks += q.trial_blocks; t.trial_cyc_heap += q.trial_cyc_heap; t.trial_cyc_fallback += q.trial_cyc_fallback;
    t.trial_symbols += q.trial_symbols; t.n_trials_replayed += q.n_trials_replayed; t.n_replay_checked += q.n_replay_checked;
    t.n_trials_duplicate += q.n_trials_duplicate; t.n_trials_skipped += q.n_trials_skipped;
    tch = std::max(tch, p->t_chains); ttr = std::max(ttr, p->t_trials); tap = std::max(tap, p->t_apply);
    for (int k = 0; k < 3; k++) for (int l = 0; l < 10; l++) for (int i = 0; i < 14; i++) kind[k][l][i] += p->kind[k][l][i];
  }
  if (timing_on()) {
    std::fprintf(stderr, "atz: sweep host: chains %.1f ms (incl. kernels), trials %.1f ms (incl. kernels), apply %.1f ms, total %.1f ms\n",
                 tch, ttr, tap, ms_since(R.t0));
    std::fprintf(stderr, "atz: device/pinned allocations so far: %llu allocs, %llu frees, %.1f ms in them\n",
                 (unsigned long long)g_dev.n_alloc.load(), (unsigned long long)g_dev.n_free.load(), g_dev.alloc_us.load() / 1e3);
    for (size_t g = 0; g < np; g++) {
      Pipe* p = c->pipes[g].get();
      std::fprintf(stderr, "atz: pipe %zu: %llu copy calls %.1f ms, %llu syncs %.1f ms\n", g, (unsigned long long)p->n_copy,
                   p->t_copy, (unsigned long long)p->n_sync, p->t_sync);
      static const char* phn[Pipe::NPH] = {"list", "tables-enq", "tables-sync", "replay-plan", "plan-rest", "order",
                                           "match-jobs", "match-launch", "trial-launch", "results", "apply", "diffs", "account"};
      std::string line;
      char b[96];
      for (int i = 0; i < Pipe::NPH; i++) {
        std::snprintf(b, sizeof b, " %s %.1f(%.1f)", phn[i], p->ph[i], p->ph_wait[i]);
        line += b;
      }
      std::fprintf(stderr, "atz: pipe %zu host phases ms (waiting):%s\n", g, line.c_str());
    }
    uint64_t nb = 0, nn = 0;
    for (size_t g = 0; g < np; g++) {
      Pipe* p = c->pipes[g].get();
      nb += p->diag_builds;
      for (uint16_t v : p->diag_need) nn += (uint64_t)__builtin_popcount(v);
      p->diag_builds = 0;
      p->diag_need.clear();
    }
    std::fprintf(stderr, "atz: bucket builds %llu, (stream, memLevel) pairs a table-reading trial used %llu; bucket cache "
                 "%.2f GB allocated, %.2f GB served from released tables; saved sequences %.2f GB; device peak %.2f GB\n",
                 (unsigned long long)nb, (unsigned long long)nn, c->chain_arena.total / 1e9, c->chain_arena.reused / 1e9,
                 c->rp_arena.total / 1e9, g_dev.peak.load() / 1e9);
  }
  if (timing_level() >= 3) {
    std::vector<uint64_t> path(n, 0), ntr(n, 0);
    for (size_t g = 0; g < np; g++) {
      Pipe* p = c->pipes[g].get();
      for (size_t s2 = 0; s2 < p->diag_path.size() && s2 < n; s2++) { path[s2] += p->diag_path[s2]; ntr[s2] += p->diag_ntr[s2]; }
      p->diag_path.clear();
      p->diag_ntr.clear();
    }
    std::vector<uint32_t> ord(n);
    for (size_t s2 = 0; s2 < n; s2++) ord[s2] = (uint32_t)s2;
    std::sort(ord.begin(), ord.end(), [&](uint32_t a, uint32_t b) { return path[a] > path[b]; });
    if (n) {
      auto q = [&](double f) { return path[ord[std::min(n - 1, (size_t)(f * (double)n))]] / 1e5; };
      std::fprintf(stderr, "atz: per-stream trial time (ms, summed over its trials): max %.2f p1 %.2f p5 %.2f p10 %.2f p50 %.2f\n",
                   q(0.0), q(0.01), q(0.05), q(0.10), q(0.5));
      for (size_t i = 0; i < n && i < 8; i++)
        std::fprintf(stderr, "atz:   stream %u: %.2f ms over %llu trials, I=%llu C=%llu ident %llu type %d phase %u\n", ord[i],
                     path[ord[i]] / 1e5, (unsigned long long)ntr[ord[i]], (unsigned long long)c->recs[ord[i]].infl_len,
                     (unsigned long long)c->recs[ord[i]].comp_len, (unsigned long long)ss[ord[i]].ident, c->recs[ord[i]].type,
                     ss[ord[i]].phase);
    }
  }
  if (timing_level() >= 3) {
    std::vector<std::pair<uint32_t, int>> ev;
    for (size_t g = 0; g < np; g++) {
      Pipe* p = c->pipes[g].get();
      for (auto& e : p->diag_rt) { ev.push_back({e.first, 1}); ev.push_back({e.second, -1}); }
      p->diag_rt.clear();
    }
    if (!ev.empty()) {
      std::sort(ev.begin(), ev.end());
      const uint32_t t0 = ev.front().first, t1 = ev.back().first;
      double area = 0;
      int cur = 0, peak = 0;
      uint32_t last = t0;
      std::vector<double> bin((size_t)((t1 - t0) / 500000u) + 1, 0.0);
      for (auto& e : ev) {
        for (uint64_t a = last - t0; a < (uint64_t)(e.first - t0);) {
          const uint64_t b = std::min<uint64_t>(e.first - t0, (a / 500000u + 1u) * 500000u);
          bin[(size_t)(a / 500000u)] += (double)cur * (double)(b - a);
          a = b;
        }
        area += (double)cur * (e.first - last);
        cur += e.second;
        peak = std::max(peak, cur);
        last = e.first;
      }
      std::fprintf(stderr, "atz: trials in flight: mean %.0f over %.1f ms, peak %d; per 5 ms:", area / std::max<uint32_t>(1, t1 - t0),
                   (t1 - t0) / 1e5, peak);
      for (double v : bin) std::fprintf(stderr, " %.0f", v / 500000.0);
      std::fprintf(stderr, "\n");
    }
  }
  if (timing_on())
    for (int k = 0; k < 3; k++)
      for (int l = 0; l < 10; l++) {
        const uint64_t* gk = kind[k][l];
        if (!gk[0]) continue;
        std::fprintf(stderr, "atz: kind %d level %d: trials %llu cyc %.3fT (tree %.3fT [heap %.3fT scan %.3fT] emit %.3fT [send %.3fT] fb %.3fT) "
                     "parsed %.1f MB syms %.1f M cyc/byte %.0f\n", k, l, (unsigned long long)gk[0], gk[1] / 1e12,
                     gk[2] / 1e12, gk[4] / 1e12, gk[8] / 1e12, gk[3] / 1e12, gk[9] / 1e12, gk[5] / 1e12, gk[6] / 1e6, gk[7] / 1e6,
                     gk[6] ? (double)gk[1] / gk[6] : 0.0);
        std::fprintf(stderr, "atz:     window phases: refill %.3fT steps %.3fT path %.3fT tally+flush %.3fT\n",
                     gk[10] / 1e12, gk[11] / 1e12, gk[12] / 1e12, gk[13] / 1e12);
      }
  for (size_t s = 0; s < n; s++) {
    StreamState& st = ss[s];
    const uint64_t C = c->recs[s].comp_len;
    st.recomp = (C - st.ident) <= c->o.recomp_tresh && st.ident > 0;
  }
  c->stats.sweep_ms = ms_since(R.t0);
  return 0;
}

struct SweepGuard {
  atz_ctx* c;
  SweepRun& R;
  ~SweepGuard() { if (R.running) sweep_close(c, R, true); }
};

static void strategy_list(std::vector<uint32_t>& l, int type, uint32_t mask) {
  if (type >= 24) return;
  const int w = 10 + type / 4;
  static const int mo[9] = {8, 9, 7, 6, 5, 4, 3, 2, 1};
  auto add = [&](uint32_t strat, int chi, int clo) {
    if (!((mask >> strat) & 1u)) return;
    for (int m : mo)
      for (int cl = chi; cl >= clo; cl--) l.push_back((strat << 24) | pk(cl, w, m));
  };
  switch (type % 4) {
    case 0: add(3, 6, 6); add(2, 6, 6); break;
    case 1: add(1, 5, 4); break;
    case 2: add(1, 6, 6); break;
    default: add(1, 9, 7); break;
  }
}

static void raw_list(std::vector<uint32_t>& l, int type);
static int ext_pass(atz_ctx* c, const uint8_t* d_file, std::vector<StreamState>& ss, bool raw) {
  const auto t0 = std::chrono::steady_clock::now();
  const size_t n = ss.size();
  struct Ext {
    std::vector<uint32_t> list;
    uint32_t best = 0;
    uint64_t ident = 0;
    bool done = false;
    std::vector<uint32_t> rawdiff;
    std::vector<uint8_t> diffval;
  };
  std::vector<Ext> ex(n);
  std::vector<uint32_t> todo;
  size_t longest = 0;
  for (size_t s = 0; s < n; s++) {
    if (ss[s].recomp || c->recs[s].infl_len >= (1ull << 31)) continue;
    if (raw) raw_list(ex[s].list, c->recs[s].type);
    else strategy_list(ex[s].list, c->recs[s].type, c->strat_mask);
    if (ex[s].list.empty()) continue;
    todo.push_back((uint32_t)s);
    longest = std::max(longest, ex[s].list.size());
  }
  if (todo.empty()) return 0;
  if (int r = ensure_pipes(c, 1)) return r;
  HIPCHK(hipStreamSynchronize(c->st));
  Pipe* p = c->pipes[0].get();
  c->pipes_running = 1;
  p->mw_cap = mw_cap_for(todo.size());
  p->stopj_cur = nullptr;
  const atz_stats_t before = p->stats;
  const SweepOpts so{c->o.recomp_tresh, c->o.sizediff_tresh, c->o.shortcut_len, c->o.mismatch_tol};
  const uint64_t budget = cap_bytes(ROUND_BUDGET_BYTES);
  RuleTally tally;
  for (size_t j = 0; j < longest; j++) {
    std::vector<uint32_t> act;
    for (uint32_t s : todo)
      if (!ex[s].done && j < ex[s].list.size()) act.push_back(s);
    if (act.empty()) break;
    for (size_t a0 = 0; a0 < act.size();) {
      size_t a1 = a0;
      uint64_t bytes = 0;
      while (a1 < act.size() && (a1 == a0 || bytes <= budget)) {
        const uint32_t s = act[a1], q = ex[s].list[j];
        const uint64_t len = c->recs[s].infl_len;
        bytes += 9 * len + 4 * sym_words(p, 2, q & 0xff, len) + bound(len, (int)((q >> 8) & 0xff), (int)(q & 0xff)) + 4096;
        a1++;
      }
      std::vector<std::pair<uint32_t, int>> need;
      for (size_t a = a0; a < a1; a++) {
        const uint32_t q = ex[act[a]].list[j];
        if (raw ? ((q >> 16) & 0xff) > 0 : (q >> 24) == 1) need.push_back({act[a], (int)(q & 0xff)});
      }
      if (int r = private_chains(c, p, need)) return r;
      TrialBatch B;
// ... 1213 lines not shown
```

antiz_amd/csrc/atz_device.h:

```cpp
#pragma once
#include <stdint.h>

#ifndef ATZ_INF_CLOCKS
#define ATZ_INF_CLOCKS 0
#endif

namespace atz {

struct InfJob {
  uint64_t in_off;
  uint64_t in_len;
  uint64_t out_off;
  uint64_t out_cap;
};
static constexpr uint64_t NO_OUT = ~0ull;
static constexpr uint64_t ARENA_OUT = ~1ull;
static constexpr uint64_t ARENA_NONE = ~0ull;

enum : uint32_t { INF_END = 0, INF_ERROR = 1, INF_NEED = 2, INF_RETRY = 3 };

static constexpr uint32_t INF_HINT_NOSHORT = 1u << 31;
static constexpr uint32_t INF_HINT_MLEV_SHIFT = 27;

struct InfRes {
  uint32_t status;
  uint32_t err;
  uint64_t consumed;
  uint64_t produced;
  uint64_t arena_off;
#if ATZ_INF_CLOCKS
  uint64_t cyc, nlit, nmatch;
  uint64_t cyc_copy, cyc_flush;
  uint64_t nfar, cyc_far;
  uint64_t nblk, cyc_hdr, nlong;
#endif
};

enum : uint8_t {
  TM_FULL = 1,
  TM_RAW = 2,
  TM_SAVE = 4,
  TM_REPLAY = 8,
  TM_CHECKED = 16,
  TM_SAVE_TAB = 32,
  TM_RP_SYMS = TM_SAVE | TM_REPLAY,
  TM_RP_TAB = TM_CHECKED | TM_SAVE_TAB,
};
enum : uint32_t {
  TH_STRAT = 3,
  TH_WAITS = 4,
  TH_DUP = 8,
};
struct Trial {
  uint32_t stream;
  uint8_t clevel, window, memlevel, mode;
  uint64_t best_ident;
  uint64_t out_off;
  uint64_t out_cap;
  uint64_t sym_off;
  uint64_t chain_off;
  uint64_t r_off;
  uint64_t x_lim;
  uint64_t rp_syms;
  uint64_t rp_tab;
  uint32_t rp_nsym, rp_flags;
  uint32_t spec_j, host;
};
static_assert(sizeof(Trial) == 96, "the trial kernels load this layout");
static inline bool tm_unchecked_replay(uint8_t mode) { return (mode & (TM_REPLAY | TM_CHECKED)) == TM_REPLAY; }

struct MatchJob {
  uint64_t infl_off, n;
  uint64_t chain_off;
  uint64_t r_off;
  uint64_t p0, p1;
  uint32_t level, window;
  uint32_t fast, memlevel;
};

struct StreamDev {
  uint64_t orig_off;
  uint64_t infl_off;
  uint64_t comp_len;
  uint64_t infl_len;
};

struct TrialRes {
  uint32_t state;
  uint32_t flags;
  uint64_t out_len;
  uint64_t ident;
  uint64_t symbols;
  uint64_t parsed;
  uint64_t fallbacks;
  uint64_t cyc_total, cyc_tree, cyc_emit, blocks;
  uint64_t cyc_heap, cyc_fallback;
  uint64_t cyc_scan, cyc_send;
  uint64_t cyc_sec[4];
  uint32_t saved_syms;
  uint32_t saved_flags;
  uint32_t reads_max;
  uint32_t rt0, rt1;
  uint32_t pad_;
};
enum : uint32_t {
  TR_FULL = 0,
  TR_SHORTCUT = 1,
  TR_SIZEDIFF = 2,
  TR_CANT_BEAT = 3,
  TR_OVERFLOW = 4,
  TR_NEED_R = 5,
  TR_SKIPPED = 6,
};

struct SweepOpts {
  uint64_t recomp_tresh, sizediff_tresh, shortcut_len, mismatch_tol;
};

__device__ __forceinline__ uint32_t wave_incl_scan(uint32_t v) {
  int x = (int)v;
  x += __builtin_amdgcn_update_dpp(0, x, 0x111, 0xf, 0xf, false);
  x += __builtin_amdgcn_update_dpp(0, x, 0x112, 0xf, 0xf, false);
  x += __builtin_amdgcn_update_dpp(0, x, 0x114, 0xf, 0xf, false);
  x += __builtin_amdgcn_update_dpp(0, x, 0x118, 0xf, 0xf, false);
  x += __builtin_amdgcn_update_dpp(0, x, 0x142, 0xa, 0xf, false);
  x += __builtin_amdgcn_update_dpp(0, x, 0x143, 0xc, 0xf, false);
  return (uint32_t)x;
}

}
```

antiz_amd/csrc/k_deflate.hip:

```cpp
#include <hip/hip_runtime.h>
#include "atz_device.h"

#define LDS __attribute__((address_space(3)))
#define CONSTANT __attribute__((address_space(4)))
#define GLOBAL __attribute__((address_space(1)))

#ifndef ATZ_VISITED_CHECK
#define ATZ_VISITED_CHECK 1
#endif
#ifndef ATZ_VISITED_MAX
#define ATZ_VISITED_MAX 8
#endif
#ifndef ATZ_NOSLIDE_PATH
#define ATZ_NOSLIDE_PATH 1
#endif
#ifndef ATZ_STEP_SPLIT
#define ATZ_STEP_SPLIT 0
#endif
#ifndef ATZ_STEP_CLOCKS
#define ATZ_STEP_CLOCKS 0
#endif
#if ATZ_STEP_CLOCKS
#define STEP_CLOCK() clock64()
#else
// ... 364 lines not shown
    const uint32_t b4 = 4u * (uint32_t)tid;
    uint32_t c4[4], s = 0;
#pragma unroll
    for (int u = 0; u < 4; u++) { c4[u] = cnt[b4 + u]; s += c4[u]; }
    const uint32_t incl = wave_incl_scan(s);
    if (lane == 63) wtot[wave] = incl;
    __syncthreads();
    const uint32_t off = (uint32_t)__builtin_amdgcn_readlane((int)wave_incl_scan(lane < wave ? wtot[lane] : 0u), 63);
    uint32_t e = off + incl - s;
#pragma unroll
    for (int u = 0; u < 4; u++) { cnt[b4 + u] = (uint16_t)e; e += c4[u]; }
    __syncthreads();
#pragma unroll 1
    for (uint32_t c = 0; c < MAXC; c++) {
      if (t0 + 64 * c >= t1) break;
      const uint32_t i = t0 + 64 * c + (uint32_t)lane;
      const bool valid = i < t1;
      const uint32_t d = (hashv(c) >> shift) & dmask;
      const uint64_t pm = digit_peers(d, valid, bits);
      const uint32_t base = valid ? (uint32_t)cnt[d * BSORT_W + wave] : 0u;
      if (valid) {
        Y[base + (uint32_t)__popcll(pm & lt)] = (uint16_t)posv(c);
        if ((pm & lt) == 0) cnt[d * BSORT_W + wave] = (uint16_t)(base + (uint32_t)__popcll(pm));
      }
    }
  };
  static_assert(256 * BSORT_W == 4 * BSORT_THREADS, "the scan takes 4 counters per thread");
  if (hbits <= 8) {
    pass(0, hbits);
  } else {
    pass(0, hbits - 8);
    reload();
    pass(hbits - 8, 8);
  }
  reload();
  uint32_t* const last_start = wtot;
  if (tid == 0) dmax = 0;
  uint32_t carry = 0, mine = 0;
  bool before = true;
  uint32_t lead = 0;
  uint32_t hprev = t0 > 0 && t0 < t1 ? bhash(in, (uint32_t)Y[t0 - 1], hshift, hmask) : ~0u;
#pragma unroll 1
  for (uint32_t c = 0; c < MAXC; c++) {
    if (t0 + 64 * c >= t1) break;
    const uint32_t i0 = t0 + 64 * c;
    const uint32_t i = i0 + (uint32_t)lane;
    const bool valid = i < t1;
    const uint32_t h = hashv(c);
    const uint32_t up = (uint32_t)__shfl_up((int)h, 1, 64);
    const uint32_t hp = lane ? up : hprev;
    hprev = (uint32_t)__builtin_amdgcn_readlane((int)h, 63);
    const bool first = valid && (i == 0 || hp != h);
    if (valid) bpos[i] = posv(c) | (first ? BUCKET_FIRST : 0u);
    if (depth_out) {
      const uint64_t fm = __ballot(first);
      const uint64_t le = lane == 63 ? ~0ull : ((2ull << lane) - 1ull);
      const uint64_t at = fm & le;
      const uint32_t st = at ? i0 + (63u - (uint32_t)__builtin_clzll(at)) : carry;
      if (valid && (at || !before)) mine = mine > i - st ? mine : i - st;
      if (valid && !at && before) lead = i - t0 + 1;
      if (fm) { carry = i0 + 63u - (uint32_t)__builtin_clzll(fm); before = false; }
    }
  }
  if (depth_out && lane == 0) last_start[wave] = before ? ~0u : carry;
  __syncthreads();
#pragma unroll 1
  for (uint32_t c = 0; c < MAXC; c++) {
    if (t0 + 64 * c >= t1) break;
    const uint32_t i = t0 + 64 * c + (uint32_t)lane;
    if (i < t1) Y[posv(c)] = (uint16_t)i;
  }
  if (depth_out) {
    uint32_t prev = ~0u;
    for (int w = wave - 1; w >= 0 && prev == ~0u; w--) prev = last_start[w];
    uint32_t lm = 0;
    if (lead && prev != ~0u) lm = t0 + lead - 1u - prev;
    lm = lm > mine ? lm : mine;
    for (int d = 32; d >= 1; d >>= 1) { const uint32_t o = __shfl_xor(lm, d, 64); lm = lm > o ? lm : o; }
    if (lane == 0 && lm) atomicMax(&dmax, lm);
  }
  __syncthreads();
  for (uint32_t q = tid; q < nh; q += BSORT_THREADS) sidx[q] = Y[q];
  if (depth_out && tid == 0) depth_out[jb.dslot] = dmax;
}

static constexpr uint32_t BDEPTH_THREADS = 1024;
__global__ __launch_bounds__(BDEPTH_THREADS) void k_bucket_depth(const uint8_t* __restrict__ infl,
                                                                const ChainJob* __restrict__ jobs, uint32_t njobs,
                                                                uint32_t* __restrict__ depth_out) {
  extern __shared__ uint32_t dyn_lds[];
  __shared__ uint32_t dmax;
  const uint32_t j = blockIdx.x;
  if (j >= njobs) return;
  const int tid = threadIdx.x;
  const ChainJob jb = jobs[j];
  const uint8_t* in = infl + jb.infl_off;
  const uint32_t n = (uint32_t)jb.n;
  const uint32_t hbits = jb.memlevel + 7, hmask = (1u << hbits) - 1, hshift = (hbits + 2) / 3;
  const uint32_t nw = 1u << (hbits - 1);
  LDS uint32_t* cnt = (LDS uint32_t*)dyn_lds;
  for (uint32_t w = tid; w < nw; w += BDEPTH_THREADS) cnt[w] = 0;
  if (tid == 0) dmax = 0;
  __syncthreads();
  const uint32_t nh = n >= 3 ? n - 2 : 0;
  uint32_t mine = 0;
  for (uint32_t p = tid; p < nh; p += BDEPTH_THREADS) {
    const uint32_t h = (((uint32_t)in[p] << (2 * hshift)) ^ ((uint32_t)in[p + 1] << hshift) ^ in[p + 2]) & hmask;
    const uint32_t sh = 16u * (h & 1u);
    const uint32_t old = __hip_atomic_fetch_add(&cnt[h >> 1], 1u << sh, __ATOMIC_RELAXED, __HIP_MEMORY_SCOPE_WORKGROUP);
    const uint32_t c = ((old >> sh) & 0xffffu) + 1u;
    mine = mine > c ? mine : c;
  }
  for (int d = 32; d >= 1; d >>= 1) { const uint32_t o = __shfl_xor(mine, d, 64); mine = mine > o ? mine : o; }
  if ((tid & 63) == 0 && mine) atomicMax(&dmax, mine);
  __syncthreads();
  if (tid == 0) depth_out[jb.dslot] = dmax ? dmax - 1u : 0u;
}

#ifndef ATZ_HOLE_SLOTS
#define ATZ_HOLE_SLOTS 256
#endif
static constexpr uint32_t HOLE_SLOTS_M = ATZ_HOLE_SLOTS;
static_assert(HOLE_SLOTS_M <= 2048 && (HOLE_SLOTS_M & (HOLE_SLOTS_M - 1)) == 0, "slot field is 11 bits of the match entry");

template <typename P>
__device__ __forceinline__ void load16(P in32, uint32_t x, uint32_t v[4]) {
  const uint32_t w = x >> 2, sh = x & 3;
  const uint32_t a0 = in32[w], a1 = in32[w + 1], a2 = in32[w + 2], a3 = in32[w + 3], a4 = in32[w + 4];
  v[0] = __builtin_amdgcn_alignbyte(a1, a0, sh);
  v[1] = __builtin_amdgcn_alignbyte(a2, a1, sh);
  v[2] = __builtin_amdgcn_alignbyte(a3, a2, sh);
  v[3] = __builtin_amdgcn_alignbyte(a4, a3, sh);
}
template <typename P>
__device__ __forceinline__ uint32_t match16(P in32, uint32_t a, uint32_t b, const uint32_t* pb, int) {
  uint32_t va[4], vb[4];
  load16(in32, a, va);
  if (pb) { vb[0] = pb[0]; vb[1] = pb[1]; vb[2] = pb[2]; vb[3] = pb[3]; }
  else load16(in32, b, vb);
#pragma unroll
  for (int k = 0; k < 4; k++) {
    const uint32_t x = va[k] ^ vb[k];
    if (x) return 4 * k + ((uint32_t)__builtin_ctz(x) >> 3);
  }
  return 16;
}

template <typename P>
__device__ __forceinline__ void match_positions(const MatchJob& jb, const uint8_t* __restrict__ in, P in32,
                                                const uint32_t* __restrict__ chains, uint2* __restrict__ R) {
  const uint32_t n = (uint32_t)jb.n, npad = (n + 63) & ~63u;
  const uint32_t* sidx = chains + jb.chain_off;
  const uint32_t* bpos = sidx + npad;
  uint2* r = R + jb.r_off;
  const uint32_t B = c_cfg[jb.level][3], nice = c_cfg[jb.level][2], Bq = B >> 2;
  const uint32_t maxdist = (1u << jb.window) - 262;
  const uint32_t hbits = jb.memlevel + 7u, hmask = (1u << hbits) - 1u, hshift = (hbits + 2u) / 3u;
  for (uint32_t p = (uint32_t)jb.p0 + threadIdx.x; p < (uint32_t)jb.p1; p += 256) {
    uint32_t bf = 2, df = 0, bq = 2, dq = 0, valid = 0, slot = 0, budget_out = 0;
    uint32_t reach = p;
    const uint32_t s0 = in[p];
    if (p + 3 <= n) {
      const uint32_t s1 = in[p + 1];
      slot = (((s0 << (2 * hshift)) ^ (s1 << hshift) ^ (uint32_t)in[p + 2]) & hmask) & (HOLE_SLOTS_M - 1);
      const uint32_t lim = p > maxdist ? p - maxdist : 0u;
      uint32_t idx = sidx[p];
      uint32_t e = bpos[idx];
      if (!(e & BUCKET_FIRST)) {
        e = bpos[--idx];
        uint32_t cur = e & ~BUCKET_FIRST;
        if (cur >= 1 && cur + maxdist >= p) {
          valid = 1;
          const uint32_t left = n - p;
          const uint32_t cap = left < 258 ? left : 258u;
          const uint32_t nn = nice < cap ? nice : cap;
          uint32_t pv[4];
          load16(in32, p, pv);
          for (uint32_t i = 0;;) {
            reach = cur;
            const bool more = !(e & BUCKET_FIRST);
            const uint32_t en = more ? bpos[idx - 1] : 0u;
            uint32_t len = match16(in32, cur, p, pv, 0);
            if (len == 16)
              while (len < cap) {
                const uint32_t l2 = match16(in32, cur + len, p + len, nullptr, 0);
                len += l2;
                if (l2 < 16) break;
              }
            if (len > cap) len = cap;
            if (len > bf) {
              bf = len; df = p - cur;
              if (i < Bq) { bq = len; dq = df; }
              if (len >= nn) break;
            }
            if (++i == B) {
              budget_out = (more && (en & ~BUCKET_FIRST) > lim) ? 1u : 0u;
              break;
            }
            if (!more) break;
            e = en;
            idx--;
            cur = e & ~BUCKET_FIRST;
            if (cur <= lim) break;
          }
        }
      }
    }
    uint2 o;
    o.x = (bf > 2 ? (bf << 23) | (df << 8) : 0u) | s0;
    if (jb.fast) o.y = ((p - reach) << 16) | (budget_out << 12) | (slot << 1) | valid;
    else o.y = (bq > 2 ? (bq << 23) | (dq << 8) : 0u) | valid;
    r[p] = o;
  }
}

__global__ __launch_bounds__(256) void k_match(const uint8_t* __restrict__ infl, const uint32_t* __restrict__ chains,
                                              uint2* __restrict__ R, const MatchJob* __restrict__ jobs) {
  const MatchJob jb = jobs[blockIdx.x];
  const uint8_t* in = infl + jb.infl_off;
  match_positions(jb, in, reinterpret_cast<const uint32_t*>(in), chains, R);
}

static constexpr uint32_t PREV_NIL = 0xffffu;
#ifndef ATZ_MATCH_THREADS
#define ATZ_MATCH_THREADS 1024
#endif
static constexpr uint32_t MATCH_THREADS = ATZ_MATCH_THREADS;
struct LdsWin {
  const LDS uint32_t* p;
  uint32_t off;
  __device__ __forceinline__ uint32_t operator[](uint32_t w) const { return p[w - off]; }
};
__global__ __launch_bounds__(MATCH_THREADS) void k_match_lds(const uint8_t* __restrict__ infl, const uint32_t* __restrict__ chains,
                                                  uint2* __restrict__ R, const MatchJob* __restrict__ jobs) {
  extern __shared__ uint32_t dyn_lds[];
  const MatchJob jb = jobs[blockIdx.x];
  const uint8_t* in = infl + jb.infl_off;
  const uint32_t* g32 = reinterpret_cast<const uint32_t*>(in);
  const uint32_t n = (uint32_t)jb.n, npad = (n + 63) & ~63u;
  const uint32_t* sidx = chains + jb.chain_off;
  const uint32_t* bpos = sidx + npad;
  const uint32_t maxdist = (1u << jb.window) - 262;
  const uint32_t lo = (uint32_t)jb.p0 > maxdist ? ((uint32_t)jb.p0 - maxdist) & ~3u : 0u;
  const uint32_t w0 = lo >> 2;
  const uint64_t want = jb.p1 + 258 + 24;
  const uint32_t nw = (uint32_t)(((want < n ? want : n) + 3) >> 2) - w0;
  LDS uint32_t* l32 = (LDS uint32_t*)dyn_lds;
  LDS uint16_t* prv = (LDS uint16_t*)(l32 + nw + 8);
  for (uint32_t w = threadIdx.x; w < nw + 8; w += MATCH_THREADS) l32[w] = w < nw ? g32[w0 + w] : 0u;
  const uint32_t nh = n >= 3 ? n - 2 : 0;
  const uint32_t P = (uint32_t)jb.p1 < nh ? (uint32_t)jb.p1 : nh;
  auto pred = [&](uint32_t a, uint32_t b) -> uint16_t {
    const uint32_t pq = b & ~BUCKET_FIRST;
    return ((a & BUCKET_FIRST) || pq < lo) ? (uint16_t)PREV_NIL : (uint16_t)(pq - lo);
  };
  if (P > lo && 4 * (P - lo) >= nh) {
    for (uint32_t i0 = 0; i0 < nh; i0 += 8 * MATCH_THREADS) {
      uint32_t a[8], b[8];
#pragma unroll
      for (int u = 0; u < 8; u++) {
        const uint32_t i = i0 + MATCH_THREADS * u + threadIdx.x;
        a[u] = i < nh ? bpos[i] : BUCKET_FIRST | 0x7fffffffu;
        b[u] = (i < nh && i) ? bpos[i - 1] : 0u;
      }
#pragma unroll
      for (int u = 0; u < 8; u++) {
        const uint32_t q = a[u] & ~BUCKET_FIRST;
        if (q >= lo && q < P) prv[q - lo] = pred(a[u], b[u]);
      }
    }
  } else {
    for (uint32_t q0 = lo; q0 < P; q0 += 8 * MATCH_THREADS) {
      uint32_t ix[8], a[8], b[8];
#pragma unroll
      for (int u = 0; u < 8; u++) { const uint32_t q = q0 + MATCH_THREADS * u + threadIdx.x; ix[u] = q < P ? sidx[q] : 1u; }
#pragma unroll
      for (int u = 0; u < 8; u++) { a[u] = bpos[ix[u]]; b[u] = ix[u] ? bpos[ix[u] - 1] : 0u; }
#pragma unroll
      for (int u = 0; u < 8; u++) {
        const uint32_t q = q0 + MATCH_THREADS * u + threadIdx.x;
        if (q < P) prv[q - lo] = pred(a[u], b[u]);
      }
    }
  }
  __syncthreads();
  const LdsWin in32{l32, w0};
  auto byte = [&](uint32_t x) -> uint32_t { return (in32[x >> 2] >> (8 * (x & 3))) & 0xffu; };
  uint2* r = R + jb.r_off;
  const uint32_t B = c_cfg[jb.level][3], nice = c_cfg[jb.level][2], Bq = B >> 2;
  const uint32_t hbits = jb.memlevel + 7u, hmask = (1u << hbits) - 1u, hshift = (hbits + 2u) / 3u;
  for (uint32_t p = (uint32_t)jb.p0 + threadIdx.x; p < (uint32_t)jb.p1; p += MATCH_THREADS) {
    uint32_t bf = 2, df = 0, bq = 2, dq = 0, valid = 0, slot = 0, budget_out = 0;
    uint32_t reach = p;
    const uint32_t s0 = byte(p);
    if (p + 3 <= n) {
      slot = (((s0 << (2 * hshift)) ^ (byte(p + 1) << hshift) ^ byte(p + 2)) & hmask) & (HOLE_SLOTS_M - 1);
      const uint32_t lim = p > maxdist ? p - maxdist : 0u;
      const uint32_t h0 = prv[p - lo];
      uint32_t cur = h0 + lo;
      if (h0 != PREV_NIL && cur >= 1 && cur + maxdist >= p) {
        valid = 1;
        const uint32_t left = n - p;
        const uint32_t cap = left < 258 ? left : 258u;
        const uint32_t nn = nice < cap ? nice : cap;
        uint32_t pv[4];
        load16(in32, p, pv);
        for (uint32_t i = 0;;) {
          reach = cur;
          const uint32_t nr = prv[cur - lo];
          const bool more = nr != PREV_NIL;
          const uint32_t nx = nr + lo;
          uint32_t len = match16(in32, cur, p, pv, 0);
          if (len == 16)
            while (len < cap) {
              const uint32_t l2 = match16(in32, cur + len, p + len, nullptr, 0);
              len += l2;
              if (l2 < 16) break;
            }
          if (len > cap) len = cap;
          if (len > bf) {
            bf = len; df = p - cur;
            if (i < Bq) { bq = len; dq = df; }
            if (len >= nn) break;
          }
          if (++i == B) {
            budget_out = (more && nx > lim) ? 1u : 0u;
            break;
          }
          if (!more) break;
          cur = nx;
          if (cur <= lim) break;
        }
      }
    }
    uint2 o;
    o.x = (bf > 2 ? (bf << 23) | (df << 8) : 0u) | s0;
    if (jb.fast) o.y = ((p - reach) << 16) | (budget_out << 12) | (slot << 1) | valid;
    else o.y = (bq > 2 ? (bq << 23) | (dq << 8) : 0u) | valid;
    r[p] = o;
  }
}

static constexpr int NLC = 286, NDC = 30, NBLC = 19, HEAPN = 2 * NLC + 1;
static constexpr uint32_t LOOKMIN = 262;
static constexpr uint32_t BITMAP_BITS = 32768;
static constexpr uint32_t HOLE_SLOTS = HOLE_SLOTS_M;

struct TreeWork {
  uint32_t heap[HEAPN + 1];
  uint16_t bl_count[16];
  uint32_t blc32[16];
};

struct TreeScratch {
  uint16_t anc[2][HEAPN];
  uint8_t dep[2][HEAPN];
  uint16_t freq[NLC];
};

struct BitOut {
  GLOBAL uint8_t* out;
  uint64_t cap;
  uint64_t pos;
  uint64_t bb;
  uint32_t bc;
  uint32_t raw;
  const GLOBAL uint8_t* orig;
  uint64_t clen;
  uint64_t shortcut;
  uint64_t eq_all;
  uint64_t eq_sc;
  int overflow;
  uint64_t cyc_tree, cyc_emit, blocks;
  uint64_t cyc_heap, cyc_scan, cyc_send;
};

static constexpr uint32_t STAGE_WORDS = 196;
struct BlockFreq {
  uint32_t lfreq2[(NLC + 1) / 2];
  uint32_t dfreq2[NDC / 2];
};
struct TreeCodes {
  uint16_t lcode[NLC]; uint8_t llen[NLC + 2];
  uint16_t dcode[NDC]; uint8_t dlen[NDC + 2];
  uint16_t bcode[NBLC]; uint8_t blen[NBLC + 2];
  uint32_t bfreq[NBLC];
  TreeWork w;
};
struct TrialShared {
  BitOut b;
  BlockFreq f;
  TreeCodes k;
  uint64_t stop_at;
  uint32_t stop_j, pad_;
};

template <uint32_t INS>
struct TrialSharedFast {
  static constexpr uint32_t INS_BITS = INS;
  TrialShared t;
  uint64_t ring[512];
  uint32_t ins[INS / 32];
  uint32_t holes[HOLE_SLOTS];
};

static constexpr uint32_t RING_SLOW = 512;
struct TrialSharedSlow {
  TrialShared t;
  uint64_t ring[RING_SLOW];
};
static_assert(sizeof(TreeScratch) <= RING_SLOW * sizeof(uint64_t), "tree scratch overlays the ring");
static_assert(offsetof(BitOut, cyc_scan) == offsetof(BitOut, cyc_heap) + 8, "block_trees' cyc[0], cyc[1]");
static_assert(STAGE_WORDS * 4 <= RING_SLOW * sizeof(uint64_t), "emission staging overlays the ring");

#ifndef ATZ_MW_F
#define ATZ_MW_F 3
#endif
static constexpr int MW_F = ATZ_MW_F;
struct MWSlot {
  BlockFreq f;
  int64_t block_start;
  uint64_t p, S;
  uint32_t last_lit, sbase, last, seq;
};
struct MWFlusher {
  TreeCodes k;
  TreeScratch sc;
  uint64_t cyc_tree, cyc_emit;
  uint64_t cyc_heap, cyc_scan;
};
static_assert(offsetof(MWFlusher, cyc_scan) == offsetof(MWFlusher, cyc_heap) + 8, "block_trees' cyc[0], cyc[1]");
struct MWCtl {
  uint32_t next_emit;
  uint32_t stop;
  uint32_t parse_done, nblocks;
  uint32_t state, hazard;
};
struct MWPart {
  MWSlot slot[MW_F];
  MWFlusher fl[MW_F];
  MWCtl ctl;
};
template <uint32_t INS>
struct TrialSharedFastMW {
  static constexpr uint32_t INS_BITS = INS;
  TrialShared t;
  uint64_t ring[512];
  uint32_t ins[INS / 32];
  uint32_t holes[HOLE_SLOTS];
  MWPart mw;
};
struct TrialSharedSlowMW {
  TrialShared t;
  uint64_t ring[RING_SLOW];
  MWPart mw;
};
static_assert(sizeof(TrialSharedFastMW<BITMAP_BITS>) <= 64 * 1024 && sizeof(TrialSharedSlowMW) <= 64 * 1024, "static LDS of a block");
template <typename T> struct HasMW { static constexpr bool value = false; };
template <uint32_t INS> struct HasMW<TrialSharedFastMW<INS>> { static constexpr bool value = true; };
template <> struct HasMW<TrialSharedSlowMW> { static constexpr bool value = true; };
__device__ __forceinline__ uint32_t ld_acq(const LDS uint32_t& x) {
  return uni(__hip_atomic_load(&x, __ATOMIC_ACQUIRE, __HIP_MEMORY_SCOPE_WORKGROUP));
}
__device__ __forceinline__ void st_rel(LDS uint32_t& x, uint32_t v, int lane) {
  if (lane == 0) __hip_atomic_store(&x, v, __ATOMIC_RELEASE, __HIP_MEMORY_SCOPE_WORKGROUP);
}

struct SweepArgs {
  const uint8_t* file;
  const uint8_t* infl;
  const uint32_t* chains;
  const uint2* R;
  const StreamDev* streams;
  const Trial* trials;
  TrialRes* res;
  uint32_t* stopj;
  uint8_t* out;
  uint32_t* syms;
  const uint32_t* adler;
  SweepOpts o;
  uint32_t ntrials;
};

__device__ inline uint64_t wsum64(uint64_t v) {
  for (int d = 32; d >= 1; d >>= 1) {
    uint32_t lo = __shfl_xor((uint32_t)v, d, 64), hi = __shfl_xor((uint32_t)(v >> 32), d, 64);
    v += ((uint64_t)hi << 32) | lo;
  }
  return v;
}

__device__ inline void emit_bytes_from_stage(LDS BitOut& b, const LDS uint32_t* stage, uint32_t nb, int lane) {
  uint32_t eqa = 0, eqs = 0;
// ... 1879 lines not shown
```

include/atz_accel.h:

```cpp
#ifndef ATZ_ACCEL_H
#define ATZ_ACCEL_H
#include <stdint.h>
#ifdef __cplusplus
extern "C" {
#endif

typedef struct atz_ctx atz_ctx_t;

typedef struct {
    uint64_t recomp_tresh;
    uint64_t sizediff_tresh;
    uint64_t shortcut_len;
    uint64_t mismatch_tol;
    uint64_t chunksize;
    int32_t  brute_window;
    int32_t  device;
} atz_opts_t;

typedef struct {
    uint64_t offset;
    uint64_t comp_len;
    uint64_t infl_len;
    int32_t  type;
    uint32_t flags;
} atz_cand_t;

typedef struct {
    uint8_t  clevel, window, memlevel, recomp;
    uint32_t n_trials;
    uint64_t ident;
    int64_t  first_diff;
    uint64_t n_diff;
    uint64_t diff_index;
} atz_result_t;

typedef struct {
    uint64_t file_bytes, n_streams, n_recomp, n_trials, n_trials_shortcut, n_rounds, atz_bytes;
    uint64_t n_candidates, n_continuations, n_hazard;
    double scan_ms, sweep_ms, write_ms, total_ms;
    double k_trial_ms, k_inflate_ms, k_chains_ms, k_other_ms;
    uint64_t k_trial_launches, k_inflate_launches, k_chains_launches;
    uint64_t k_trial_alg_bytes, k_inflate_alg_bytes, k_chains_alg_bytes;
    uint64_t trial_parsed_bytes;
    double k_match_ms;
    uint64_t k_match_launches, k_match_positions;
    uint64_t n_trials_rerun;
    uint64_t n_fast_fallbacks;
    uint64_t trial_cyc_total, trial_cyc_tree, trial_cyc_emit, trial_blocks;
    uint64_t trial_cyc_heap, trial_cyc_fallback, trial_symbols;
    uint64_t n_trials_speculative;
    uint64_t n_reinflated;
    uint64_t n_inflate_retries;
    uint64_t n_trials_replayed;
    uint64_t n_replay_checked;
    uint64_t n_trials_duplicate;
    uint64_t n_fast_restarts;
    uint64_t dev_bytes_peak, dev_bytes_held;
    uint64_t n_trials_skipped;
} atz_stats_t;

enum {
    ATZ_OK = 0,
    ATZ_E_ARG = -1,
    ATZ_E_NODEV = -2,
    ATZ_E_HIP = -3,
    ATZ_E_NOMEM = -4,
    ATZ_E_REF_ABORT = -5,
    ATZ_E_REF_UB = -6,
    ATZ_E_FORMAT = -7,
    ATZ_E_INTERNAL = -8
};

int  atz_open(atz_ctx_t **ctx, const atz_opts_t *opts);
void atz_close(atz_ctx_t *ctx);
const char *atz_strerror(int err);
void atz_free(void *p);
void atz_default_opts(atz_opts_t *opts);

int atz_scan(atz_ctx_t *ctx, const uint8_t *file, uint64_t len, atz_cand_t **out, uint64_t *n);

int atz_sweep(atz_ctx_t *ctx, const atz_cand_t *cands, uint64_t n, atz_result_t *res,
              uint64_t **diff_off, uint8_t **diff_val, uint64_t *n_diffs);

int atz_precompress(atz_ctx_t *ctx, const uint8_t *file, uint64_t len, uint8_t **atz, uint64_t *atz_len,
                    atz_stats_t *stats);

int atz_precompress_device(atz_ctx_t *ctx, const uint8_t *d_file, const uint8_t *h_file, uint64_t len,
                           const uint8_t **d_atz, uint64_t *atz_len, atz_stats_t *stats);

int atz_reconstruct(atz_ctx_t *ctx, const uint8_t *atz, uint64_t len, uint8_t **out, uint64_t *out_len);

int atz_reconstruct_device(atz_ctx_t *ctx, const uint8_t *d_atz, const uint8_t *h_atz, uint64_t len,
                           const uint8_t **d_out, uint64_t *out_len);

int atz_deflate(atz_ctx_t *ctx, const uint8_t *in, uint64_t in_len, int clevel, int window, int memlevel,
                uint8_t *out, uint64_t out_cap, uint64_t *out_len);

int atz_deflate_batch(atz_ctx_t *ctx, const uint8_t *buf, uint64_t len, const uint64_t *offs, const uint64_t *lens,
                      const uint32_t *params, uint64_t n, uint8_t *out, const uint64_t *out_offs,
                      const uint64_t *out_caps, uint64_t *out_lens);

int atz_deflate_batch_ex(atz_ctx_t *ctx, const uint8_t *buf, uint64_t len, const uint64_t *offs, const uint64_t *lens,
                         const uint32_t *params, uint64_t n, uint8_t *out, const uint64_t *out_offs,
                         const uint64_t *out_caps, uint64_t *out_lens);

int atz_set_strategies(atz_ctx_t *ctx, uint32_t mask);

int atz_set_containers(atz_ctx_t *ctx, uint32_t mask);

int atz_container_anchors(atz_ctx_t *ctx, const uint8_t *file, uint64_t len, uint32_t mask, uint64_t **out,
                          uint64_t *n);

int atz_inflate_batch(atz_ctx_t *ctx, const uint8_t *buf, uint64_t len, const uint64_t *offs,
                      const uint64_t *lens, uint64_t n, uint32_t *status, uint64_t *consumed, uint64_t *produced);

int atz_shard_scan(atz_ctx_t *ctx, const uint8_t *d_file, const uint8_t *h_file, uint64_t len, int rank, int world,
                   uint8_t **blob, uint64_t *blob_len);
int atz_shard_sweep(atz_ctx_t *ctx, const uint8_t *d_file, const uint8_t *h_file, uint64_t len,
                    const uint8_t *const *blobs, const uint64_t *blob_lens, int world, uint64_t *piece_len,
                    uint8_t **recomp_flags, uint64_t *n_flags, uint64_t *n_recomp, atz_stats_t *stats);
int atz_shard_piece(atz_ctx_t *ctx, uint8_t *d_dst);
int atz_shard_assemble(atz_ctx_t *ctx, const uint8_t *d_file, uint64_t len, const uint8_t *recomp_flags,
                       uint64_t n_flags, uint64_t n_recomp, uint64_t pieces_len, uint8_t *d_atz, uint64_t cap,
                       uint64_t *atz_len);

uint64_t atz_deflate_bound(uint64_t n, int window, int memlevel);

#ifdef __cplusplus
}
#endif
#endif
```

Before: 1690.

## Share one hash-chain walk across sibling compression levels in match kernel

When a stream's parameter list has several upcoming levels with the same window and memlevel, the first match job now allocates extra result tables for up to MATCH_GROUP levels. A templated LDS match kernel walks each chain once and records per-level best matches in one pass, so later trials at those levels reuse the precomputed tables instead of launching their own match work. Trials now carry absolute table addresses, and the kernel is specialized on whether a sliding window is needed. The change adds a sibling-table arena with free lists, more register pressure from the per-level state, an optional verification path that compares against single-level walks, and a risk of wasted walks when speculative siblings are skipped.

```diff
diff --git a/antiz_amd/__init__.py b/antiz_amd/__init__.py
--- a/antiz_amd/__init__.py
+++ b/antiz_amd/__init__.py
@@ -38,7 +38,7 @@
                                    "trial_cyc_heap", "trial_cyc_fallback", "trial_symbols",
                                    "n_trials_speculative", "n_reinflated", "n_inflate_retries", "n_trials_replayed", "n_replay_checked",
                                    "n_trials_duplicate", "n_fast_restarts", "dev_bytes_peak", "dev_bytes_held",
-                                   "n_trials_skipped")]
+                                   "n_trials_skipped", "k_match_level_entries")]
 
     def as_dict(self):
         return {k: getattr(self, k) for k, _ in self._fields_}
diff --git a/antiz_amd/csrc/atz_accel.cpp b/antiz_amd/csrc/atz_accel.cpp
--- a/antiz_amd/csrc/atz_accel.cpp
+++ b/antiz_amd/csrc/atz_accel.cpp
@@ -340,6 +340,14 @@
   uint8_t rp_win[10] = {};
   bool recomp = false;
   std::vector<std::array<uint16_t, 5>> xl;
+  struct SibTab {
+    uint64_t addr = 0;
+    uint32_t extent = 0;
+    uint16_t li = 0;
+    uint8_t level = 0;
+  };
+  std::array<SibTab, MATCH_GROUP - 1> sib;
+  uint8_t sib_w = 0, sib_m = 0, sib_phase = 0;
 };
 
 
@@ -517,6 +525,7 @@
   atz_stats_t stats{};
   DBuf d_trials, d_tres, d_out, d_syms, d_R, d_mjobs, d_diffjobs, d_diffpos, d_diffval, d_diffcnt, d_djobs;
   DBuf d_stopj;
+  DBuf d_mverify, d_mvjobs, d_mvflag;
   uint32_t* stopj_cur = nullptr;
   uint32_t mw_cap = 2;
   std::vector<std::unique_ptr<DBuf>> d_chains;
@@ -525,6 +534,9 @@
   PinBuf stage;
   size_t stage_used = 0;
   uint64_t r_next = 0;
+  std::vector<StreamState>* ss_cur = nullptr;
+  bool group_walks = false;
+  std::unordered_map<uint64_t, std::vector<uint64_t>> sib_free;
   hipEvent_t ev_built = nullptr;
 
   hipStream_t pst = nullptr;
@@ -591,6 +603,8 @@
   std::vector<std::array<uint64_t, 10>> chain_off;
   DevArena chain_arena;
   DevArena rp_arena;
+  DevArena sib_arena;
+  std::atomic<uint64_t> sib_cap_hits{0};
   std::vector<std::array<RpEntry, 9>> rp_pool;
   std::mutex rp_mu;
   PinBuf depth_pin;
@@ -1679,7 +1693,19 @@
   const uint64_t lo = m.p0 > md ? (m.p0 - md) & ~3ull : 0ull;
   return std::min<uint64_t>(m.p1 + 258 + 24, m.n) - lo;
 }
-static int launch_match(atz_ctx* x, Pipe* c, const std::vector<MatchJob>& mj_in) {
+static uint32_t match_share() {
+  static const uint32_t v = [] {
+    const char* e = std::getenv("ATZ_MATCH_SHARE");
+    return e ? (uint32_t)std::max(1, std::min((int)MATCH_GROUP, std::atoi(e))) : MATCH_GROUP;
+  }();
+  return v;
+}
+static bool match_verify() {
+  const char* e = std::getenv("ATZ_MATCH_VERIFY");
+  return e && std::atoi(e) != 0;
+}
+static int verify_groups(atz_ctx* x, Pipe* c, const std::vector<MatchJob>& mj);
+static int launch_match(atz_ctx* x, Pipe* c, const std::vector<MatchJob>& mj_in, bool verify = true) {
   if (mj_in.empty()) return 0;
   static const uint64_t cls[] = {4096, 8192, 12288, 16384, 24576, 32768, 40960, 49152};
   constexpr int NC = 8;
@@ -1701,47 +1727,103 @@
     for (int k = 0; k < NC; k++) if (b <= cls[k] && (win || k < 6)) return k;
     return NC;
   };
-  auto group_of = [](int k) -> int { return k; };
-  std::vector<MatchJob> mj;
-  mj.reserve(mj0.size());
-  size_t cnt[NC + 1] = {};
-  int gmax[NC + 1];
-  for (int k = 0; k <= NC; k++) gmax[k] = -1;
-  for (const MatchJob& m : mj0) {
-    const int k = class_of(m), g = group_of(k);
-    cnt[g]++;
-    gmax[g] = std::max(gmax[g], k);
-  }
-  size_t beg[NC + 2] = {};
-  for (int k = 0; k <= NC; k++) beg[k + 1] = beg[k] + cnt[k];
-  mj.resize(mj0.size());
+  constexpr int NG = NC * (int)MATCH_GROUP + 1;
+  auto group_of = [&](const MatchJob& m) -> int {
+    const int k = class_of(m);
+    return k < NC ? k * (int)MATCH_GROUP + (int)m.nlev - 1 : NG - 1;
+  };
+  std::vector<MatchJob> mj(mj0.size());
+  size_t cnt[NG] = {}, beg[NG + 1] = {};
+  for (const MatchJob& m : mj0) cnt[group_of(m)]++;
+  for (int g = 0; g < NG; g++) beg[g + 1] = beg[g] + cnt[g];
   {
-    size_t at[NC + 1];
-    for (int k = 0; k <= NC; k++) at[k] = beg[k];
-    for (const MatchJob& m : mj0) mj[at[group_of(class_of(m))]++] = m;
+    size_t at[NG];
+    for (int g = 0; g < NG; g++) at[g] = beg[g];
+    for (const MatchJob& m : mj0) mj[at[group_of(m)]++] = m;
     auto work = [](const MatchJob& m) -> uint64_t {
-      const uint64_t chain = std::min<uint64_t>(c_cfg_host(m.level), (m.p1 >> (m.memlevel + 7)) + 1);
+      uint64_t deep = c_cfg_host(m.level);
+      for (uint32_t g = 1; g < m.nlev; g++) deep = std::max(deep, c_cfg_host(m.lev[g - 1]));
+      const uint64_t chain = std::min<uint64_t>(deep, (m.p1 >> (m.memlevel + 7)) + 1);
       return (m.p1 - m.p0) * chain;
     };
-    for (int k = 0; k <= NC; k++)
-      std::stable_sort(mj.begin() + beg[k], mj.begin() + beg[k + 1],
-                       [&](const MatchJob& a, const MatchJob& b) { return work(a) > work(b); });
+    std::vector<std::pair<uint64_t, uint32_t>> key(mj.size());
+    for (size_t i = 0; i < mj.size(); i++) key[i] = {~work(mj[i]), (uint32_t)i};
+    for (int g = 0; g < NG; g++) std::sort(key.begin() + beg[g], key.begin() + beg[g + 1]);
+    std::vector<MatchJob> sorted(mj.size());
+    for (size_t i = 0; i < mj.size(); i++) sorted[i] = mj[key[i].second];
+    mj.swap(sorted);
   }
   if (int r = upload(c, c->d_mjobs, mj.data(), mj.size() * sizeof(MatchJob))) return r;
-  for (int k = 0; k <= NC; k++) {
-    if (!cnt[k]) continue;
+  using MatchKern = void (*)(const uint8_t*, const uint32_t*, uint2*, const MatchJob*);
+  static const MatchKern lds_kern[MATCH_GROUP] = {k_match_lds<1>, k_match_lds<2>, k_match_lds<3>, k_match_lds<4>};
+  for (int g = 0; g < NG; g++) {
+    if (!cnt[g]) continue;
     kbeg(c, 4);
-    if (k < NC)
-      hipLaunchKernelGGL(k_match_lds, dim3((uint32_t)cnt[k]), dim3(MATCH_THREADS), (uint32_t)(3 * cls[gmax[k]] + 64), c->st,
-                         INFL_BASE, CHAIN_BASE, c->d_R.as<uint2>(),
-                         c->d_mjobs.as<MatchJob>() + beg[k]);
+    if (g < NG - 1)
+      hipLaunchKernelGGL(lds_kern[g % (int)MATCH_GROUP], dim3((uint32_t)cnt[g]), dim3(MATCH_THREADS),
+                         (uint32_t)(3 * cls[g / (int)MATCH_GROUP] + 64), c->st, INFL_BASE, CHAIN_BASE, c->d_R.as<uint2>(),
+                         c->d_mjobs.as<MatchJob>() + beg[g]);
     else
-      hipLaunchKernelGGL(k_match, dim3((uint32_t)cnt[k]), dim3(256), 0, c->st, INFL_BASE,
-                         CHAIN_BASE, c->d_R.as<uint2>(), c->d_mjobs.as<MatchJob>() + beg[k]);
+      hipLaunchKernelGGL(k_match, dim3((uint32_t)cnt[g]), dim3(256), 0, c->st, INFL_BASE,
+                         CHAIN_BASE, c->d_R.as<uint2>(), c->d_mjobs.as<MatchJob>() + beg[g]);
     kend(c);
     KCHECK("k_match");
   }
-  for (const MatchJob& m : mj) c->stats.k_match_positions += m.p1 - m.p0;
+  bool groups = false;
+  for (const MatchJob& m : mj) {
+    c->stats.k_match_positions += m.p1 - m.p0;
+    c->stats.k_match_level_entries += (m.p1 - m.p0) * m.nlev;
+    groups |= m.nlev > 1;
+  }
+  if (groups && verify && match_verify()) return verify_groups(x, c, mj);
+  return 0;
+}
+static int verify_groups(atz_ctx* x, Pipe* c, const std::vector<MatchJob>& mj) {
+  const uint64_t keep_p = c->stats.k_match_positions, keep_e = c->stats.k_match_level_entries;
+  constexpr uint64_t BATCH = 32ull << 20;
+  std::vector<MatchJob> vj;
+  std::vector<MatchCmp> cmp;
+  uint64_t used = 0;
+  if (int r = c->d_mvflag.reserve(64)) return r;
+  auto flush = [&]() -> int {
+    if (vj.empty()) return 0;
+    if (int r = c->d_mverify.reserve(used * sizeof(uint2) + 4096)) return r;
+    const uint64_t base = (uint64_t)(uintptr_t)c->d_mverify.p;
+    for (size_t i = 0; i < vj.size(); i++) {
+      cmp[i].b += base;
+      vj[i].tab[0] = cmp[i].b - 8 * vj[i].p0;
+    }
+    HIPCHK(hipMemsetAsync(c->d_mvflag.p, 0xff, 8, c->st));
+    if (int r = launch_match(x, c, vj, false)) return r;
+    if (int r = upload(c, c->d_mvjobs, cmp.data(), cmp.size() * sizeof(MatchCmp))) return r;
+    hipLaunchKernelGGL(k_match_cmp, dim3((uint32_t)cmp.size()), dim3(256), 0, c->st, c->d_mvjobs.as<MatchCmp>(),
+                       c->d_mvflag.as<unsigned long long>());
+    KCHECK("k_match_cmp");
+    unsigned long long f = 0;
+    HIPCHK(pipe_copy(c, &f, c->d_mvflag.p, 8, hipMemcpyDeviceToHost));
+    HIPCHK(pipe_sync(c));
+    if (f != ~0ull) {
+      const MatchCmp& q = cmp[(size_t)(f >> 32)];
+      std::fprintf(stderr, "atz: group walk differs from the single-level walk: stream %u level %u position %llu\n",
+                   q.stream, q.level, (unsigned long long)(f & 0xffffffffull));
+      return ATZ_E_INTERNAL;
+    }
+    vj.clear(); cmp.clear(); used = 0;
+    return 0;
+  };
+  for (const MatchJob& m : mj)
+    for (uint32_t g = 1; g < m.nlev; g++) {
+      const uint64_t cnt = m.p1 - m.p0;
+      if (used && used + cnt > BATCH)
+        if (int r = flush()) return r;
+      MatchJob v = m;
+      v.level = m.lev[g - 1]; v.fast = v.level <= 3; v.nlev = 1;
+      vj.push_back(v);
+      cmp.push_back(MatchCmp{m.tab[g] + 8 * m.p0, 8 * used, cnt, m.p0, m.stream, v.level});
+      used += cnt;
+    }
+  if (int r = flush()) return r;
+  c->stats.k_match_positions = keep_p; c->stats.k_match_level_entries = keep_e;
   return 0;
 }
 
@@ -1836,6 +1918,14 @@
   };
   for (size_t i = 0; i < cnt; i++)
     if (h[i].host & (TH_WAITS | TH_DUP)) return ATZ_E_INTERNAL;
+  std::vector<Trial> abs_tr;
+  if (k) {
+    abs_tr.assign(h, h + cnt);
+    const uint64_t r_base = (uint64_t)(uintptr_t)c->d_R.p >> 3;
+    for (Trial& t : abs_tr)
+      if (!(t.host & TH_TAB_ABS)) t.r_off += r_base;
+    h = abs_tr.data();
+  }
   for (size_t i = 0; i < cnt;) {
     const bool mw = mw_trial(c, k, h[i].memlevel);
     size_t j = i + 1;
@@ -1852,7 +1942,7 @@
     if (!kn) return ATZ_E_INTERNAL;
     SweepArgs A;
     A.file = d_cmp; A.infl = INFL_BASE; A.chains = CHAIN_BASE;
-    A.R = c->d_R.as<uint2>();
+    A.R = nullptr;
     A.streams = x->d_streams.as<StreamDev>(); A.trials = c->d_trials.as<Trial>() + b1;
     A.res = c->d_tres.as<TrialRes>() + b1; A.out = c->d_out.as<uint8_t>(); A.syms = c->d_syms.as<uint32_t>();
     A.adler = x->d_adler.as<uint32_t>(); A.o = so; A.ntrials = (uint32_t)n1;
@@ -1878,14 +1968,73 @@
   static const bool v = [] { const char* e = std::getenv("ATZ_EARLY"); return !e || std::atoi(e) != 0; }();
   return v;
 }
+static constexpr uint64_t SIB_ARENA_CAP = 32ull << 30;
+static uint64_t table_entries(uint64_t n) { return ((n + 63) & ~63ull) + 256; }
+static bool may_skip_table(const StreamState& st, uint32_t level, uint32_t window, uint32_t memlevel) {
+  bool maybe = false;
+  if (st.rp >= 0) maybe = ((st.rp_saved >> level) & 1u) && st.rp_win[level] == window;
+  if (!maybe && level >= 7)
+    for (const auto& r : st.xl) maybe |= r[0] == window && r[1] == memlevel && r[2] > level;
+  return maybe;
+}
+static uint64_t sib_alloc(atz_ctx* x, Pipe* c, uint64_t n) {
+  const uint64_t bytes = DevArena::cls(table_entries(n) * sizeof(uint2));
+  auto it = c->sib_free.find(bytes);
+  if (it != c->sib_free.end() && !it->second.empty()) {
+    const uint64_t a = it->second.back();
+    it->second.pop_back();
+    return a;
+  }
+  return x->sib_arena.alloc(bytes);
+}
+static void release_sibs(Pipe* c, StreamState& st, uint64_t n, uint32_t upto) {
+  for (auto& s : st.sib)
+    if (s.addr && s.li < upto) {
+      c->sib_free[DevArena::cls(table_entries(n) * sizeof(uint2))].push_back(s.addr);
+      s = StreamState::SibTab{};
+    }
+}
 static MatchJob first_match_job(atz_ctx* x, Pipe* c, int k, Trial& t) {
   const uint64_t n = x->recs[t.stream].infl_len;
-  t.r_off = c->r_next;
-  c->r_next += ((n + 63) & ~63ull) + 256;
   t.x_lim = (t.mode & TM_FULL) || (mhint_on(x) && t.memlevel == x->recs[t.stream].mhint) ? n : match_prefix(n, t.memlevel, big_sweep(x));
   MatchJob m{};
-  m.infl_off = x->infl_off[t.stream]; m.n = n; m.chain_off = t.chain_off; m.r_off = t.r_off;
+  m.infl_off = x->infl_off[t.stream]; m.n = n; m.chain_off = t.chain_off;
   m.p0 = 0; m.p1 = t.x_lim; m.level = t.clevel; m.window = t.window; m.fast = k == 1; m.memlevel = t.memlevel;
+  m.nlev = 1; m.stream = t.stream;
+  StreamState* st = c->ss_cur ? &(*c->ss_cur)[t.stream] : nullptr;
+  if (st) {
+    const bool mine = st->sib_w == t.window && st->sib_m == t.memlevel && st->sib_phase == st->phase;
+    bool any = false;
+    for (auto& s : st->sib) {
+      any |= s.addr != 0;
+      if (!mine || !s.addr || s.level != t.clevel) continue;
+      t.r_off = s.addr >> 3;
+      t.host |= TH_TAB_ABS;
+      m.tab[0] = s.addr;
+      m.p0 = std::min<uint64_t>(s.extent, t.x_lim);
+      t.x_lim = std::max<uint64_t>(s.extent, t.x_lim);
+      s.extent = (uint32_t)t.x_lim;
+      return m;
+    }
+    if (!any && c->group_walks && match_win() > 0) {
+      st->sib_w = t.window; st->sib_m = t.memlevel; st->sib_phase = (uint8_t)st->phase;
+      for (uint32_t li = st->idx + t.spec_j + 1; li < st->list->size() && m.nlev < match_share(); li++) {
+        const uint32_t p = (*st->list)[li];
+        const uint32_t lv = p >> 16;
+        if (((p >> 8) & 0xff) != t.window || (p & 0xff) != t.memlevel || lv < 1) break;
+        if (may_skip_table(*st, lv, t.window, t.memlevel)) continue;
+        const uint64_t a = sib_alloc(x, c, n);
+        if (!a) { x->sib_cap_hits++; break; }
+        st->sib[m.nlev - 1] = StreamState::SibTab{a, (uint32_t)t.x_lim, (uint16_t)li, (uint8_t)lv};
+        m.tab[m.nlev] = a;
+        m.lev[m.nlev - 1] = lv;
+        m.nlev++;
+      }
+    }
+  }
+  t.r_off = c->r_next;
+  c->r_next += table_entries(n);
+  m.r_off = t.r_off;
   return m;
 }
 static int trials_first_launch(atz_ctx* x, Pipe* c, const uint8_t* d_cmp, TrialSet& S, const SweepOpts& so,
@@ -1958,6 +2107,8 @@
       MatchJob m{};
       m.infl_off = x->infl_off[t.stream]; m.n = n; m.chain_off = t.chain_off; m.r_off = t.r_off;
       m.p0 = t.x_lim; m.p1 = n; m.level = t.clevel; m.window = t.window; m.fast = k == 1; m.memlevel = t.memlevel;
+      m.nlev = 1; m.stream = t.stream;
+      if (t.host & TH_TAB_ABS) m.tab[0] = t.r_off << 3;
       if (m.p1 > m.p0) mj.push_back(m);
       t.x_lim = n;
       again[k].push_back(t);
@@ -2277,6 +2428,8 @@
   void build_lists() {
     K = (uint32_t)std::max<size_t>(1, std::min<size_t>(32, round_target(x) / active.size()));
     c->mw_cap = mw_cap_for(std::min(x->sweep_nmax, active.size() * x->pipes_running));
+    c->ss_cur = &ss;
+    c->group_walks = match_share() > 1 && (K == 1 || active.size() * K <= 512);
     mbeg.assign(active.size() + 1, 0);
     mine.reserve(active.size() * K);
     uint64_t round_bytes = 0;
@@ -2338,10 +2491,7 @@
           const bool again = (seen[t.window & 15] >> t.clevel) & 1u;
           seen[t.window & 15] |= (uint16_t)(1u << t.clevel);
           const StreamState& st = ss[t.stream];
-          bool maybe = false;
-          if (st.rp >= 0) maybe = ((st.rp_saved >> t.clevel) & 1u) && st.rp_win[t.clevel] == t.window;
-          if (!maybe && k == 2 && t.clevel >= 7)
-            for (const auto& r : st.xl) maybe |= r[0] == t.window && r[1] == t.memlevel && r[2] > t.clevel;
+          const bool maybe = may_skip_table(st, t.clevel, t.window, t.memlevel);
           static const bool all_first = [] { const char* e = std::getenv("ATZ_DFIRST"); return e && std::atoi(e) == 0; }();
           if (maybe || all_first) {
             dfirst.push_back({t.stream, (int)t.memlevel});
@@ -2557,6 +2707,8 @@
 
   void release_done() {
     for (uint32_t s : active) {
+      StreamState& st = ss[s];
+      release_sibs(c, st, x->recs[s].infl_len, st.phase != st.sib_phase ? ~0u : st.idx);
       if (ss[s].phase != 2) continue;
       const uint64_t bytes = 8 * ((x->recs[s].infl_len + 63) & ~63ull);
       for (int m = 1; m <= 9; m++) {
@@ -2635,6 +2787,7 @@
 static int sweep_pipe(atz_ctx* x, Pipe* c, const uint8_t* d_file, std::vector<StreamState>& ss) {
   const auto t0 = std::chrono::steady_clock::now();
   std::vector<uint32_t> active;
+  c->sib_free.clear();
   const SweepOpts so{x->o.recomp_tresh, x->o.sizediff_tresh, x->o.shortcut_len, x->o.mismatch_tol};
   uint64_t rounds = 0;
   while (sched_take(x, c->id, active)) {
@@ -2644,6 +2797,8 @@
       atz_ctx* x; Pipe* c; const std::vector<StreamState>& ss; const std::vector<uint32_t>& a, &w;
       ~Give() {
         c->stopj_cur = nullptr;
+        c->ss_cur = nullptr;
+        c->group_walks = false;
         forget_tmp_chains(x, c);
         sched_give(x, c->id, ss, a, w);
       }
@@ -2741,6 +2896,8 @@
   for (auto& a : c->chain_off) a.fill(~0ull);
   c->chain_arena.reset(cap_bytes(CHAIN_CACHE_CAP));
   c->rp_arena.reset(cap_bytes(RP_ARENA_CAP));
+  c->sib_arena.reset(cap_bytes(SIB_ARENA_CAP));
+  c->sib_cap_hits = 0;
   c->rp_pool.clear();
   c->rp_pool.reserve(n_max);
   if (int r = c->depth_pin.reserve(n_max * 40 + 64)) return r;
@@ -2837,6 +2994,7 @@
     t.k_match_launches += q.k_match_launches;
     t.k_trial_alg_bytes += q.k_trial_alg_bytes; t.k_chains_alg_bytes += q.k_chains_alg_bytes;
     t.trial_parsed_bytes += q.trial_parsed_bytes; t.k_match_positions += q.k_match_positions;
+    t.k_match_level_entries += q.k_match_level_entries;
     t.n_trials_rerun += q.n_trials_rerun; t.n_fast_fallbacks += q.n_fast_fallbacks; t.n_fast_restarts += q.n_fast_restarts;
     t.trial_cyc_total += q.trial_cyc_total; t.trial_cyc_tree += q.trial_cyc_tree; t.trial_cyc_emit += q.trial_cyc_emit;
     t.trial_blocks += q.trial_blocks; t.trial_cyc_heap += q.trial_cyc_heap; t.trial_cyc_fallback += q.trial_cyc_fallback;
@@ -2876,6 +3034,8 @@
                  "%.2f GB allocated, %.2f GB served from released tables; saved sequences %.2f GB; device peak %.2f GB\n",
                  (unsigned long long)nb, (unsigned long long)nn, c->chain_arena.total / 1e9, c->chain_arena.reused / 1e9,
                  c->rp_arena.total / 1e9, g_dev.peak.load() / 1e9);
+    std::fprintf(stderr, "atz: sibling match tables %.2f GB allocated (cap %.2f GB), %llu group members dropped at the cap\n",
+                 c->sib_arena.total / 1e9, c->sib_arena.cap / 1e9, (unsigned long long)c->sib_cap_hits.load());
   }
   if (timing_level() >= 3) {
     std::vector<uint64_t> path(n, 0), ntr(n, 0);
diff --git a/antiz_amd/csrc/atz_device.h b/antiz_amd/csrc/atz_device.h
--- a/antiz_amd/csrc/atz_device.h
+++ b/antiz_amd/csrc/atz_device.h
@@ -50,6 +50,7 @@
   TH_STRAT = 3,
   TH_WAITS = 4,
   TH_DUP = 8,
+  TH_TAB_ABS = 16,
 };
 struct Trial {
   uint32_t stream;
@@ -69,6 +70,7 @@
 static_assert(sizeof(Trial) == 96, "the trial kernels load this layout");
 static inline bool tm_unchecked_replay(uint8_t mode) { return (mode & (TM_REPLAY | TM_CHECKED)) == TM_REPLAY; }
 
+static constexpr uint32_t MATCH_GROUP = 4;
 struct MatchJob {
   uint64_t infl_off, n;
   uint64_t chain_off;
@@ -76,6 +78,14 @@
   uint64_t p0, p1;
   uint32_t level, window;
   uint32_t fast, memlevel;
+  uint64_t tab[MATCH_GROUP];
+  uint32_t nlev;
+  uint32_t lev[MATCH_GROUP - 1];
+  uint32_t stream, pad_;
+};
+struct MatchCmp {
+  uint64_t a, b, n, p0;
+  uint32_t stream, level;
 };
 
 struct StreamDev {
diff --git a/antiz_amd/csrc/k_deflate.hip b/antiz_amd/csrc/k_deflate.hip
--- a/antiz_amd/csrc/k_deflate.hip
+++ b/antiz_amd/csrc/k_deflate.hip
@@ -540,7 +540,7 @@
   const uint32_t n = (uint32_t)jb.n, npad = (n + 63) & ~63u;
   const uint32_t* sidx = chains + jb.chain_off;
   const uint32_t* bpos = sidx + npad;
-  uint2* r = R + jb.r_off;
+  uint2* r = jb.tab[0] ? reinterpret_cast<uint2*>(jb.tab[0]) : R + jb.r_off;
   const uint32_t B = c_cfg[jb.level][3], nice = c_cfg[jb.level][2], Bq = B >> 2;
   const uint32_t maxdist = (1u << jb.window) - 262;
   const uint32_t hbits = jb.memlevel + 7u, hmask = (1u << hbits) - 1u, hshift = (hbits + 2u) / 3u;
@@ -614,22 +614,98 @@
 #define ATZ_MATCH_THREADS 1024
 #endif
 static constexpr uint32_t MATCH_THREADS = ATZ_MATCH_THREADS;
+template <bool WIN>
 struct LdsWin {
   const LDS uint32_t* p;
   uint32_t off;
-  __device__ __forceinline__ uint32_t operator[](uint32_t w) const { return p[w - off]; }
+  __device__ __forceinline__ uint32_t operator[](uint32_t w) const { return p[WIN ? w - off : w]; }
 };
-__global__ __launch_bounds__(MATCH_THREADS) void k_match_lds(const uint8_t* __restrict__ infl, const uint32_t* __restrict__ chains,
-                                                  uint2* __restrict__ R, const MatchJob* __restrict__ jobs) {
-  extern __shared__ uint32_t dyn_lds[];
-  const MatchJob jb = jobs[blockIdx.x];
+template <bool WIN, int G>
+__device__ __forceinline__ void match_lds_walk(const MatchJob& jb, const LdsWin<WIN> in32, const LDS uint16_t* prv, uint32_t lo,
+                                               uint2* __restrict__ R) {
+  auto byte = [&](uint32_t x) -> uint32_t { return (in32[x >> 2] >> (8 * (x & 3))) & 0xffu; };
+  const uint32_t n = (uint32_t)jb.n, maxdist = (1u << jb.window) - 262;
+  uint2* r[G];
+  uint32_t B[G], nice[G], Bq[G];
+  bool fast[G];
+#pragma unroll
+  for (int g = 0; g < G; g++) {
+    const uint32_t lv = g ? jb.lev[g - 1] : jb.level;
+    r[g] = (g || jb.tab[0]) ? reinterpret_cast<uint2*>(jb.tab[g]) : R + jb.r_off;
+    B[g] = c_cfg[lv][3]; nice[g] = c_cfg[lv][2]; Bq[g] = B[g] >> 2;
+    fast[g] = g ? lv <= 3 : jb.fast != 0;
+  }
+  const uint32_t hbits = jb.memlevel + 7u, hmask = (1u << hbits) - 1u, hshift = (hbits + 2u) / 3u;
+  for (uint32_t p = (uint32_t)jb.p0 + threadIdx.x; p < (uint32_t)jb.p1; p += MATCH_THREADS) {
+    uint32_t bf[G], df[G], ya[G], yb[G], valid = 0, slot = 0;
+#pragma unroll
+    for (int g = 0; g < G; g++) { bf[g] = 2; df[g] = 0; ya[g] = fast[g] ? p : 2u; yb[g] = 0; }
+    const uint32_t s0 = byte(p);
+    if (p + 3 <= n) {
+      slot = (((s0 << (2 * hshift)) ^ (byte(p + 1) << hshift) ^ byte(p + 2)) & hmask) & (HOLE_SLOTS_M - 1);
+      const uint32_t lim = p > maxdist ? p - maxdist : 0u;
+      const uint32_t h0 = prv[p - lo];
+      uint32_t cur = h0 + lo;
+      if (h0 != PREV_NIL && cur >= 1 && cur + maxdist >= p) {
+        valid = 1;
+        const uint32_t left = n - p;
+        const uint32_t cap = left < 258 ? left : 258u;
+        uint32_t pv[4];
+        load16(in32, p, pv);
+        uint32_t live = (1u << G) - 1u;
+        for (uint32_t i = 0;;) {
+          const uint32_t nr = prv[cur - lo];
+          const bool more = nr != PREV_NIL;
+          const uint32_t nx = nr + lo;
+          uint32_t len = match16(in32, cur, p, pv, 0);
+          if (len == 16)
+            while (len < cap) {
+              const uint32_t l2 = match16(in32, cur + len, p + len, nullptr, 0);
+              len += l2;
+              if (l2 < 16) break;
+            }
+          if (len > cap) len = cap;
+          ++i;
+#pragma unroll
+          for (int g = 0; g < G; g++) {
+            if (!(live & (1u << g))) continue;
+            if (fast[g]) ya[g] = cur;
+            if (len > bf[g]) {
+              bf[g] = len; df[g] = p - cur;
+              if (!fast[g] && i <= Bq[g]) { ya[g] = len; yb[g] = df[g]; }
+              if (len >= nice[g] || len >= cap) { live &= ~(1u << g); continue; }
+            }
+            if (i == B[g]) {
+              if (fast[g]) yb[g] = (more && nx > lim) ? 1u : 0u;
+              live &= ~(1u << g);
+            }
+          }
+          if (!live || !more) break;
+          cur = nx;
+          if (cur <= lim) break;
+        }
+      }
+    }
+#pragma unroll
+    for (int g = 0; g < G; g++) {
+      uint2 o;
+      o.x = (bf[g] > 2 ? (bf[g] << 23) | (df[g] << 8) : 0u) | s0;
+      if (fast[g]) o.y = ((p - ya[g]) << 16) | (yb[g] << 12) | (slot << 1) | valid;
+      else o.y = (ya[g] > 2 ? (ya[g] << 23) | (yb[g] << 8) : 0u) | valid;
+      r[g][p] = o;
+    }
+  }
+}
+template <bool WIN, int G>
+__device__ __forceinline__ void match_lds_job(const MatchJob& jb, const uint8_t* __restrict__ infl, const uint32_t* __restrict__ chains,
+                                              uint2* __restrict__ R, uint32_t* dyn_lds) {
   const uint8_t* in = infl + jb.infl_off;
   const uint32_t* g32 = reinterpret_cast<const uint32_t*>(in);
   const uint32_t n = (uint32_t)jb.n, npad = (n + 63) & ~63u;
   const uint32_t* sidx = chains + jb.chain_off;
   const uint32_t* bpos = sidx + npad;
   const uint32_t maxdist = (1u << jb.window) - 262;
-  const uint32_t lo = (uint32_t)jb.p0 > maxdist ? ((uint32_t)jb.p0 - maxdist) & ~3u : 0u;
+  const uint32_t lo = WIN ? ((uint32_t)jb.p0 - maxdist) & ~3u : 0u;
   const uint32_t w0 = lo >> 2;
   const uint64_t want = jb.p1 + 258 + 24;
   const uint32_t nw = (uint32_t)(((want < n ? want : n) + 3) >> 2) - w0;
@@ -672,61 +748,24 @@
     }
   }
   __syncthreads();
-  const LdsWin in32{l32, w0};
-  auto byte = [&](uint32_t x) -> uint32_t { return (in32[x >> 2] >> (8 * (x & 3))) & 0xffu; };
-  uint2* r = R + jb.r_off;
-  const uint32_t B = c_cfg[jb.level][3], nice = c_cfg[jb.level][2], Bq = B >> 2;
-  const uint32_t hbits = jb.memlevel + 7u, hmask = (1u << hbits) - 1u, hshift = (hbits + 2u) / 3u;
-  for (uint32_t p = (uint32_t)jb.p0 + threadIdx.x; p < (uint32_t)jb.p1; p += MATCH_THREADS) {
-    uint32_t bf = 2, df = 0, bq = 2, dq = 0, valid = 0, slot = 0, budget_out = 0;
-    uint32_t reach = p;
-    const uint32_t s0 = byte(p);
-    if (p + 3 <= n) {
-      slot = (((s0 << (2 * hshift)) ^ (byte(p + 1) << hshift) ^ byte(p + 2)) & hmask) & (HOLE_SLOTS_M - 1);
-      const uint32_t lim = p > maxdist ? p - maxdist : 0u;
-      const uint32_t h0 = prv[p - lo];
-      uint32_t cur = h0 + lo;
-      if (h0 != PREV_NIL && cur >= 1 && cur + maxdist >= p) {
-        valid = 1;
-        const uint32_t left = n - p;
-        const uint32_t cap = left < 258 ? left : 258u;
-        const uint32_t nn = nice < cap ? nice : cap;
-        uint32_t pv[4];
-        load16(in32, p, pv);
-        for (uint32_t i = 0;;) {
-          reach = cur;
-          const uint32_t nr = prv[cur - lo];
-          const bool more = nr != PREV_NIL;
-          const uint32_t nx = nr + lo;
-          uint32_t len = match16(in32, cur, p, pv, 0);
-          if (len == 16)
-            while (len < cap) {
-              const uint32_t l2 = match16(in32, cur + len, p + len, nullptr, 0);
-              len += l2;
-              if (l2 < 16) break;
-            }
-          if (len > cap) len = cap;
-          if (len > bf) {
-            bf = len; df = p - cur;
-            if (i < Bq) { bq = len; dq = df; }
-            if (len >= nn) break;
-          }
-          if (++i == B) {
-            budget_out = (more && nx > lim) ? 1u : 0u;
-            break;
-          }
-          if (!more) break;
-          cur = nx;
-          if (cur <= lim) break;
-        }
-      }
-    }
-    uint2 o;
-    o.x = (bf > 2 ? (bf << 23) | (df << 8) : 0u) | s0;
-    if (jb.fast) o.y = ((p - reach) << 16) | (budget_out << 12) | (slot << 1) | valid;
-    else o.y = (bq > 2 ? (bq << 23) | (dq << 8) : 0u) | valid;
-    r[p] = o;
-  }
+  match_lds_walk<WIN, G>(jb, LdsWin<WIN>{l32, w0}, prv, lo, R);
+}
+template <int G>
+__global__ __launch_bounds__(MATCH_THREADS) __attribute__((amdgpu_waves_per_eu(8, 8)))
+void k_match_lds(const uint8_t* __restrict__ infl, const uint32_t* __restrict__ chains, uint2* __restrict__ R,
+                 const MatchJob* __restrict__ jobs) {
+  extern __shared__ uint32_t dyn_lds[];
+  const MatchJob jb = jobs[blockIdx.x];
+  if (jb.p0 > (1ull << jb.window) - 262) match_lds_job<true, G>(jb, infl, chains, R, dyn_lds);
+  else match_lds_job<false, G>(jb, infl, chains, R, dyn_lds);
+}
+
+__global__ __launch_bounds__(256) void k_match_cmp(const MatchCmp* __restrict__ jobs, unsigned long long* __restrict__ flag) {
+  const MatchCmp j = jobs[blockIdx.x];
+  const unsigned long long* a = reinterpret_cast<const unsigned long long*>(j.a);
+  const unsigned long long* b = reinterpret_cast<const unsigned long long*>(j.b);
+  for (uint64_t i = threadIdx.x; i < j.n; i += 256)
+    if (a[i] != b[i]) atomicMin(flag, ((unsigned long long)blockIdx.x << 32) | (j.p0 + i));
 }
 
 static constexpr int NLC = 286, NDC = 30, NBLC = 19, HEAPN = 2 * NLC + 1;
diff --git a/include/atz_accel.h b/include/atz_accel.h
--- a/include/atz_accel.h
+++ b/include/atz_accel.h
@@ -57,6 +57,7 @@
     uint64_t n_fast_restarts;
     uint64_t dev_bytes_peak, dev_bytes_held;
     uint64_t n_trials_skipped;
+    uint64_t k_match_level_entries;
 } atz_stats_t;
 
 enum {
```

Result: slower. 1642 (-2.8%).
